# aleCombi/Hedgehog.jl

Hardware: AMD Instinct MI355X
Metric: MC path-steps/sec (Heston Euler-Maruyama, 1e6 paths x 252 steps per GPU) (higher is better)
Workload: dtype f64

## Files before the change

hedgehog.jl_amd/_ffi.py:

```python
from __future__ import annotations

import ctypes as C
import os

HH_MAX_PARTIALS = 8
HH_LSM_PHASE_POW, HH_LSM_PHASE_INIT, HH_LSM_PHASE_STEP = 1, 2, 3
HH_TILE_PATHS = 256
HH_ACC_LEN = 16
HH_MAX_MODELS = 16
HH_ACC_SUM, HH_ACC_SUMSQ, HH_ACC_DSUM, HH_ACC_NPATHS = 0, 1, 2, 10

HH_LOGNORMAL, HH_HESTON = 0, 1
HH_EULER_MARUYAMA, HH_EXACT_LAW, HH_BROADIE_KAYA = 0, 1, 2
HH_NOISE_GENERATE, HH_NOISE_REPLAY = 0, 1
HH_REPLAY_TILE_MAJOR, HH_REPLAY_PATH_MAJOR = 0, 1
HH_PATH_SPOT, HH_PATH_LOG = 0, 1

HH_OK, HH_ERR_INVALID, HH_ERR_UNSUPPORTED, HH_ERR_HIP, HH_ERR_NOMEM, HH_ERR_RCCL, HH_ERR_DEVICE_TIMEOUT = 0, -1, -2, -3, -4, -5, -6
HH_MGPU_AUTO, HH_MGPU_HOST_SUM, HH_MGPU_RCCL = 0, 1, 2
HH_MGPU_REDUCE_HOST, HH_MGPU_REDUCE_RCCL = 0, 1
HH_MGPU_OPT_ENQUEUE = 1
HH_MGPU_ENQUEUE_SERIAL, HH_MGPU_ENQUEUE_THREADS = 0, 1

_dp = C.POINTER(C.c_double)


class hh_model(C.Structure):
    _fields_ = [(n, C.c_double) for n in
                ("S0", "V0", "kappa", "theta", "sigma", "rho", "r_drift", "discount", "T", "strike",
                 "cp")] + \
               [(n, _dp) for n in
                ("dS0", "dV0", "dkappa", "dtheta", "dsigma", "dr_drift", "ddiscount", "dstrike")]


class hh_config(C.Structure):
    _fields_ = [
        ("dynamics", C.c_int32), ("strategy", C.c_int32), ("antithetic", C.c_int32),
        ("em_split", C.c_int32), ("compat_sqrt_alpha", C.c_int32), ("noise_mode", C.c_int32),
        ("replay_layout", C.c_int32), ("seeds_on_device", C.c_int32),
        ("replay_on_device", C.c_int32), ("terminal_on_device", C.c_int32),
        ("n_steps", C.c_uint32), ("n_partials", C.c_uint32),
        ("n_paths", C.c_uint64), ("path_offset", C.c_uint64),
        ("seeds", C.c_void_p), ("replay", C.c_void_p),
        ("bk_n_sigma", C.c_double), ("bk_cf_tol", C.c_double), ("bk_atol", C.c_double),
        ("bk_moment_h", C.c_double),
        ("bk_newton_maxiter", C.c_int32), ("bk_bisect_maxiter", C.c_int32),
        ("bk_root_form", C.c_int32), ("bk_bracket_form", C.c_int32), ("bk_caps", C.c_int32), ("reserved0", C.c_int32),
        ("seeds_len", C.c_uint64), ("replay_len", C.c_uint64),
    ]


class hh_result(C.Structure):
    _fields_ = [
        ("price", C.c_double), ("std_error", C.c_double),
        ("sum_payoff", C.c_double), ("sumsq_payoff", C.c_double),
        ("dprice", C.c_double * HH_MAX_PARTIALS),
        ("n_paths_done", C.c_uint64),
        ("bk_newton_fail", C.c_uint64), ("bk_bisect_fallback", C.c_uint64),
        ("bk_maxguess_fallback", C.c_uint64), ("bk_cf_terms", C.c_uint64),
        ("kernel_ms", C.c_double), ("total_ms", C.c_double),
    ]


class hh_lsm_result(C.Structure):
    _fields_ = [("price", C.c_double), ("std_error", C.c_double), ("n_paths_total", C.c_uint64),
                ("rows_regressed", C.c_uint32), ("rows_skipped", C.c_uint32),
                ("kernel_ms", C.c_double), ("total_ms", C.c_double),
                ("form", C.c_int32), ("persistent_fallbacks", C.c_int32)]


HH_BK_ROOT_SECANT, HH_BK_ROOT_ORDER2 = 0, 1
HH_BK_BRACKET_MIDPOINT, HH_BK_BRACKET_ROOTS = 0, 1
HH_BK_CAPS_AS_WRITTEN, HH_BK_CAPS_ROOTS_DEFAULT = 0, 1
HH_OPT_LSM_FORM = 1
HH_OPT_BK_TERM_CACHE = 2
HH_OPT_GRID_FORM = 3
HH_OPT_LSM_SPIN_TICKS = 4
HH_OPT_FUSE_REDUCE = 5
HH_OPT_GRID_ORDER = 6
HH_OPT_FINISH_SPIN_TICKS = 7
HH_OPT_FINISH_TILE_FIRST = 8
HH_GRID_FORM_PER_DATE, HH_GRID_FORM_BATCHED = 0, 1
HH_CM_GRAD_LEN = 8
HH_LSM_FORM_PER_DATE, HH_LSM_FORM_PERSISTENT, HH_LSM_FORM_AUTO = 0, 1, 2
HH_CRR_MAX_STEPS, HH_CRR_FORM_A_MAX_STEPS = 32768, 2047
HH_CRR_EUROPEAN, HH_CRR_AMERICAN_FORWARD, HH_CRR_AMERICAN_SPOT = 0, 1, 2


class HedgehogMCError(RuntimeError):
    def __init__(self, code: int, msg: str):
        super().__init__(f"hedgehog_mc error {code}: {msg}")
        self.code = code


LIB_PATH = os.environ.get("HEDGEHOG_MC_LIB") or os.path.join(
    os.path.dirname(os.path.abspath(__file__)), "lib", "libhedgehog_mc.so")

_vp = C.c_void_p
SYMBOLS = [
    ("hh_abi_version", C.c_int, []),
    ("hh_ctx_create", C.c_int, [C.POINTER(_vp), C.c_int]),
    ("hh_ctx_destroy", None, [_vp]),
    ("hh_ctx_set_stream", C.c_int, [_vp, _vp]),
    ("hh_ctx_reset_stream", C.c_int, [_vp]),
    ("hh_last_error", C.c_char_p, [_vp]),
    ("hh_ctx_set_option", C.c_int, [_vp, C.c_int32, C.c_int64]),
    ("hh_ctx_check_last", C.c_int, [_vp]),
    ("hh_mc_solve", C.c_int, [_vp, C.POINTER(hh_model), C.POINTER(hh_config), C.POINTER(hh_result), _vp]),
    ("hh_mc_accumulate", C.c_int, [_vp, C.POINTER(hh_model), C.POINTER(hh_config), _vp, _vp]),
    ("hh_mc_solve_multi", C.c_int, [_vp, C.POINTER(hh_model), C.c_uint32, C.POINTER(hh_config), C.POINTER(hh_result), _vp]),
    ("hh_mc_accumulate_multi", C.c_int, [_vp, C.POINTER(hh_model), C.c_uint32, C.POINTER(hh_config), _vp, _vp]),
    ("hh_mc_finalize", C.c_int, [C.POINTER(hh_model), C.POINTER(hh_config), _vp, C.POINTER(hh_result)]),
    ("hh_mc_accumulate_basket", C.c_int, [_vp, C.POINTER(hh_model), C.POINTER(hh_config), _vp, _vp, C.c_uint32, _vp, _vp]),
    ("hh_mc_solve_basket", C.c_int, [_vp, C.POINTER(hh_model), C.POINTER(hh_config), _vp, _vp, C.c_uint32, _vp, _vp]),
    ("hh_carr_madan", C.c_int, [_vp, C.POINTER(hh_model), C.c_int32, C.c_int32, C.c_double, C.c_double, C.POINTER(C.c_double)]),
    ("hh_carr_madan_basket", C.c_int, [_vp, C.POINTER(hh_model), C.c_int32, C.c_int32, C.c_double, C.c_double,
                                       _vp, _vp, _vp, _vp, _vp, C.c_uint32, _vp]),
    ("hh_carr_madan_basket_grad", C.c_int, [_vp, C.POINTER(hh_model), C.c_int32, C.c_int32, C.c_double,
                                            C.c_double, _vp, _vp, _vp, _vp, _vp, C.c_uint32, _vp, _vp]),
    ("hh_crr_solve", C.c_int, [_vp, C.c_int32, C.c_uint32, _vp, _vp, _vp, _vp, _vp, _vp, _vp, C.c_uint32, _vp, _vp]),
    ("hh_lsm_grid_elems", C.c_size_t, [C.c_uint64, C.c_uint32, C.c_int32]),
    ("hh_lsm_solve", C.c_int, [_vp, C.POINTER(hh_model), C.POINTER(hh_config), C.c_int32, C.c_double, C.POINTER(hh_lsm_result), _vp, _vp, _vp]),
    ("hh_lsm_solve_grid", C.c_int, [_vp, C.POINTER(hh_model), _vp, C.c_uint64, C.c_uint32, C.c_int32, C.c_double, C.POINTER(hh_lsm_result), _vp, _vp]),
    ("hh_heston_exact_grid", C.c_int, [_vp, C.POINTER(hh_model), C.POINTER(hh_config), _vp, _vp, C.c_int32, C.POINTER(hh_result)]),
    ("hh_euler_grid", C.c_int, [_vp, C.POINTER(hh_model), C.POINTER(hh_config), C.c_int32, _vp, _vp, C.c_int32, C.POINTER(hh_result)]),
    ("hh_lsm_solve_euler", C.c_int, [_vp, C.POINTER(hh_model), C.POINTER(hh_config), C.c_int32, C.c_int32, C.c_double,
                                     C.POINTER(hh_lsm_result), _vp, _vp, _vp]),
    ("hh_lsm_shard_xchg_elems", C.c_size_t, [C.c_uint32, C.c_int32]),
    ("hh_lsm_shard_begin", C.c_int, [_vp, C.POINTER(hh_model), C.POINTER(hh_config), C.c_int32, C.c_double, _vp]),
    ("hh_lsm_shard_phase", C.c_int, [_vp, C.c_int32, C.c_uint32, _vp, _vp]),
    ("hh_lsm_shard_finish", C.c_int, [_vp, _vp, _vp, _vp, _vp, C.POINTER(C.c_uint32), C.POINTER(C.c_uint32)]),
    ("hh_lsm_finalize", C.c_int, [_vp, C.POINTER(hh_lsm_result)]),
    ("hh_lsm_debug_read", C.c_int, [_vp, C.c_uint64, C.c_uint32, C.c_int32, _vp]),
    ("hh_replay_elems", C.c_size_t, [C.c_uint64, C.c_uint32, C.c_int32]),
    ("hh_replay_pack", C.c_int, [_vp, C.c_int32, C.c_uint64, C.c_uint32, _vp, C.c_int32, _vp]),
    ("hh_wiener_fill", C.c_int, [_vp, C.c_int32, C.c_double, C.c_double, C.c_uint32, C.c_uint64, _vp, C.c_int32, _vp]),
    ("hh_seeds_fingerprint", C.c_uint64, [_vp, C.c_uint64]),
    ("hh_seeds_cache", C.c_int, [_vp, _vp, C.c_uint64, C.c_uint64, C.POINTER(_vp)]),
    ("hh_seeds_cache_stats", C.c_int, [_vp, C.POINTER(C.c_uint64), C.POINTER(C.c_uint64), C.POINTER(C.c_uint64)]),
    ("hh_device_malloc", C.c_int, [_vp, C.c_size_t, C.POINTER(_vp)]),
    ("hh_device_free", C.c_int, [_vp, _vp]),
    ("hh_memcpy_h2d", C.c_int, [_vp, _vp, _vp, C.c_size_t]),
    ("hh_memcpy_d2h", C.c_int, [_vp, _vp, _vp, C.c_size_t]),
    ("hh_ctx_synchronize", C.c_int, [_vp]),
    ("hh_ctx_enable_timing", C.c_int, [_vp, C.c_int32]),
    ("hh_ctx_read_timings", C.c_int, [_vp, _vp, C.c_int32, C.POINTER(C.c_int32)]),
    ("hh_bk_decisions", C.c_int, [_vp, C.c_uint64, _vp, _vp]),
    ("hh_mgpu_create", C.c_int, [C.POINTER(_vp), C.POINTER(C.c_int), C.c_int, C.c_int]),
    ("hh_mgpu_destroy", None, [_vp]),
    ("hh_mgpu_last_error", C.c_char_p, [_vp]),
    ("hh_mgpu_n_devices", C.c_int, [_vp]),
    ("hh_mgpu_reduce_mode", C.c_int, [_vp]),
    ("hh_mgpu_ctx", _vp, [_vp, C.c_int]),
    ("hh_mgpu_selftest", C.c_int, [_vp, C.POINTER(C.c_int32), C.POINTER(C.c_int32)]),
    ("hh_mgpu_rccl_info", C.c_int, [_vp, C.c_char_p, C.c_size_t, C.POINTER(C.c_int32), C.POINTER(C.c_int32)]),
    ("hh_mgpu_set_option", C.c_int, [_vp, C.c_int32, C.c_int64]),
    ("hh_mgpu_enqueue_stats", C.c_int, [_vp, _vp, C.POINTER(C.c_double)]),
    ("hh_mgpu_shard_range", None, [C.c_uint64, C.c_int, C.c_int, C.c_int, C.POINTER(C.c_uint64), C.POINTER(C.c_uint64)]),
    ("hh_mgpu_solve", C.c_int, [_vp, C.POINTER(hh_model), C.POINTER(hh_config), C.POINTER(hh_result), _vp]),
    ("hh_mgpu_solve_shards", C.c_int, [_vp, C.POINTER(hh_model), C.POINTER(hh_config), C.POINTER(hh_result), _vp]),
    ("hh_mgpu_solve_basket", C.c_int, [_vp, C.POINTER(hh_model), C.POINTER(hh_config), _vp, _vp, C.c_uint32, _vp]),
    ("hh_mgpu_solve_multi", C.c_int, [_vp, C.POINTER(hh_model), C.c_uint32, C.POINTER(hh_config), C.POINTER(hh_result)]),
    ("hh_mgpu_lsm_solve", C.c_int, [_vp, C.POINTER(hh_model), C.POINTER(hh_config), C.c_int32, C.c_double,
                                    C.POINTER(hh_lsm_result), _vp, _vp]),
# ... 324 lines not shown
```

hedgehog.jl_amd/csrc/hh_api.hip:

```cpp
#include <cmath>
#include <cstdarg>
#include <cstdio>
#include <cstring>
#include <mutex>
#include <vector>

#include "hh_kernels.h"

#include "hh_ctx.h"

namespace {

const char* const kNoCtx = "hedgehog_mc: no context";

int ncomp_of(int dynamics) { return dynamics == HH_HESTON ? 2 : 1; }

constexpr uint64_t kMaxPaths = (1ull << 32) - 256;
constexpr uint32_t kMaxEulerSteps = 4u * 65535u;
constexpr uint32_t kMaxGridSteps = 65534u;

static bool bk_law_ok(const hh_model* m, double dt) {
  const double s2 = m->sigma * m->sigma;
  const double d = 4.0 * m->kappa * m->theta / s2;
  if (!(d >= 1e-8 && d <= 1e6)) return false;
  const double em1 = -std::expm1(-m->kappa * dt);
  const double lam_per_v = 4.0 * m->kappa * std::exp(-m->kappa * dt) / (s2 * em1);
  const double cscale = s2 * em1 / (4.0 * m->kappa);
  const double nuk = 4.0 * m->kappa * std::exp(-0.5 * m->kappa * dt) / s2 / em1;
  return std::isfinite(lam_per_v) && lam_per_v >= 0.0 && std::isfinite(cscale) && cscale > 0.0 &&
         std::isfinite(nuk) && nuk > 0.0 && std::isfinite(m->kappa * (1.0 + std::exp(-m->kappa * dt)) / em1);
}

int validate(hh_ctx* ctx, const hh_model* m, const hh_config* c) {
  if (!m || !c) return fail(ctx, HH_ERR_INVALID, "model/config is NULL");
  if (c->n_paths == 0) return fail(ctx, HH_ERR_INVALID, "n_paths must be >= 1");
  if (c->n_paths > kMaxPaths)
    return fail(ctx, HH_ERR_INVALID, "n_paths too large (max 2^32 - 256 per call; shard the ensemble)");
  if (c->strategy == HH_EULER_MARUYAMA && c->n_steps > kMaxEulerSteps)
    return fail(ctx, HH_ERR_INVALID, "n_steps too large (max %u)", kMaxEulerSteps);
  if (c->n_partials > HH_MAX_PARTIALS)
    return fail(ctx, HH_ERR_INVALID, "n_partials %u > HH_MAX_PARTIALS", c->n_partials);
  const bool logn = c->dynamics == HH_LOGNORMAL, hest = c->dynamics == HH_HESTON;
  if (!logn && !hest) return fail(ctx, HH_ERR_INVALID, "unknown dynamics %d", c->dynamics);
  const bool ok = (logn && (c->strategy == HH_EULER_MARUYAMA || c->strategy == HH_EXACT_LAW)) ||
                  (hest && (c->strategy == HH_EULER_MARUYAMA || c->strategy == HH_BROADIE_KAYA));
  if (!ok)
    return fail(ctx, HH_ERR_UNSUPPORTED, "no simulation method for dynamics %d with strategy %d",
                c->dynamics, c->strategy);
  if (!(m->S0 > 0.0) || !std::isfinite(m->S0)) return fail(ctx, HH_ERR_INVALID, "S0 must be > 0");
  if (!(m->T > 0.0) || !std::isfinite(m->T)) return fail(ctx, HH_ERR_INVALID, "T must be > 0");
  if (m->cp != 1.0 && m->cp != -1.0) return fail(ctx, HH_ERR_INVALID, "cp must be +1 or -1");
  if (hest && !(std::fabs(m->rho) <= 1.0)) return fail(ctx, HH_ERR_INVALID, "|rho| must be <= 1");
  if (!std::isfinite(m->sigma) || !std::isfinite(m->r_drift) || !std::isfinite(m->discount) ||
      !std::isfinite(m->strike) ||
      (hest && (!std::isfinite(m->V0) || !std::isfinite(m->kappa) || !std::isfinite(m->theta))))
    return fail(ctx, HH_ERR_INVALID, "model scalars must be finite");
  if (c->strategy == HH_EULER_MARUYAMA && c->n_steps == 0)
    return fail(ctx, HH_ERR_INVALID, "n_steps must be >= 1 for EulerMaruyama");
  if (c->strategy == HH_BROADIE_KAYA) {
    if (c->antithetic)
      return fail(ctx, HH_ERR_UNSUPPORTED, "HestonBroadieKaya has no antithetic form");
    if (c->n_partials)
      return fail(ctx, HH_ERR_UNSUPPORTED, "HestonBroadieKaya does not carry dual partials");
    if (m->sigma == 0.0 || m->kappa == 0.0 || !(m->V0 > 0.0))
      return fail(ctx, HH_ERR_INVALID, "HestonBroadieKaya needs sigma != 0, kappa != 0, V0 > 0");
    if ((c->bk_root_form != HH_BK_ROOT_SECANT && c->bk_root_form != HH_BK_ROOT_ORDER2) ||
        (c->bk_bracket_form != HH_BK_BRACKET_MIDPOINT && c->bk_bracket_form != HH_BK_BRACKET_ROOTS) ||
        (c->bk_caps != HH_BK_CAPS_AS_WRITTEN && c->bk_caps != HH_BK_CAPS_ROOTS_DEFAULT))
      return fail(ctx, HH_ERR_INVALID, "bk_root_form, bk_bracket_form, bk_caps: 0 or 1 each (hedgehog_mc.h)");
    if (!bk_law_ok(m, m->T))
      return fail(ctx, HH_ERR_INVALID, "HestonBroadieKaya needs 1e-8 <= d = 4 kappa theta / sigma^2 <= 1e6 "
                                       "(Bessel order d/2 - 1 strictly above -1, tables up to order 5e5) and "
                                       "finite transition constants (|kappa T| < 700)");
  }
  const bool euler = c->strategy == HH_EULER_MARUYAMA;
  if (c->noise_mode == HH_NOISE_REPLAY) {
    if (!c->replay) return fail(ctx, HH_ERR_INVALID, "REPLAY needs a replay buffer");
    if (((uintptr_t)c->replay & 15u) != 0)
      return fail(ctx, HH_ERR_INVALID, "replay buffer must be 16-byte aligned");
    if (c->replay_len) {
      uint64_t need = c->n_paths;
      if (c->strategy == HH_BROADIE_KAYA) need = 3 * c->n_paths;
      if (euler)
        need = c->replay_layout == HH_REPLAY_PATH_MAJOR
                   ? c->n_paths * (uint64_t)c->n_steps * (uint64_t)ncomp_of(c->dynamics)
                   : (uint64_t)hh::tiles_for(c->n_paths) * c->n_steps * ncomp_of(c->dynamics) *
                         hh::kTile;
      if (c->replay_len < need)
        return fail(ctx, HH_ERR_INVALID, "replay buffer holds %llu elements, %llu needed",
                    (unsigned long long)c->replay_len, (unsigned long long)need);
    }
  } else if (c->noise_mode == HH_NOISE_GENERATE) {
    if (!c->seeds) return fail(ctx, HH_ERR_INVALID, "GENERATE needs seeds");
    const uint64_t need = euler ? c->n_paths : 1;
    if (c->seeds_len && c->seeds_len < need)
      return fail(ctx, HH_ERR_INVALID, "Number of seeds (%llu) must be >= number of trajectories (%llu)",
                  (unsigned long long)c->seeds_len, (unsigned long long)need);
  } else {
    return fail(ctx, HH_ERR_INVALID, "unknown noise_mode %d", c->noise_mode);
  }
  return HH_OK;
}

int ensure_poisoned(hh_ctx* ctx, size_t need) {
  if (need <= ctx->frecords_cap) return HH_OK;
  int rc = ensure(ctx, ctx->frecords, ctx->frecords_cap, need);
  if (rc) return rc;
  static_assert((hh::kPoison >> 32) == (hh::kPoison & 0xffffffffull), "hipMemsetD32 writes the pattern");
  HH_HIP(ctx, hipMemsetD32Async((hipDeviceptr_t)ctx->frecords, (int)(hh::kPoison & 0xffffffffull),
                                ctx->frecords_cap * 2, ctx->stream));
  return HH_OK;
}

constexpr uint32_t kFuseAutoMaxRecords = 512, kFuseAutoMinSteps = 32;
bool fuse_for(const hh_ctx* ctx, const hh_config* c) {
  if (ctx->fuse_reduce != 2) return ctx->fuse_reduce == 1;
  return hh::sim_records(*c) <= kFuseAutoMaxRecords || (c->strategy == HH_EULER_MARUYAMA && c->n_steps >= kFuseAutoMinSteps);
}

void fused_controls(const hh_ctx* ctx, hh::DevicePtrs& p) {
  p.finish_state = ctx->finish_state;
  p.finish_spin_ticks = ctx->finish_spin_ticks;
  p.finish_tile_first = ctx->finish_tile_first;
}

int recover_finish(hh_ctx* ctx) {
  unsigned int state = 0;
  HH_HIP(ctx, hipStreamSynchronize(ctx->stream));
  HH_HIP(ctx, hipMemcpy(&state, ctx->finish_state, sizeof(state), hipMemcpyDeviceToHost));
  if (state == 0u) return HH_OK;
  if (ctx->frecords_cap)
    HH_HIP(ctx, hipMemsetD32Async((hipDeviceptr_t)ctx->frecords, (int)(hh::kPoison & 0xffffffffull),
                                  ctx->frecords_cap * 2, ctx->stream));
  HH_HIP(ctx, hipMemsetAsync(ctx->finish_state, 0, 2 * sizeof(unsigned int), ctx->stream));
  HH_HIP(ctx, hipStreamSynchronize(ctx->stream));
  const long long ticks = ctx->finish_spin_ticks < 0 ? (long long)hh::kFinishSpinTicksDefault : ctx->finish_spin_ticks;
  return fail(ctx, HH_ERR_DEVICE_TIMEOUT,
              "the record reduction inside a simulation kernel gave up: a workgroup's record had not arrived after %lld "
              "ticks of the 100 MHz clock (a queue preempted for that long, or a workgroup that died); the sums of that "
              "solve, and of solves queued behind it, are lost — the context's record buffer has been reset and the "
              "context can be used again", ticks);
}

int finalize_failed(hh_ctx* ctx, int rc) {
  const int rf = recover_finish(ctx);
  return rf ? rf : fail(ctx, rc, "finalize failed: the accumulator holds no trajectories");
}

size_t replay_elems(uint64_t n_paths, uint32_t n_steps, int dynamics) {
  return (size_t)hh::tiles_for(n_paths) * n_steps * ncomp_of(dynamics) * hh::kTile;
}

int solve_times(hh_ctx* ctx, const WallClock& clock, double* kernel_ms, double* total_ms) {
  float ms = 0.f;
  HH_HIP(ctx, hipEventElapsedTime(&ms, ctx->ev0, ctx->ev1));
  *kernel_ms = ms;
  *total_ms = clock.ms();
  return HH_OK;
}

void payoff_moments(const double* acc, double n, double* mean, double* var) {
  *mean = acc[HH_ACC_SUM] / n;
  *var = n > 1.0 ? (acc[HH_ACC_SUMSQ] - n * *mean * *mean) / (n - 1.0) : 0.0;
  if (!(*var > 0.0)) *var = 0.0;
}

}

extern "C" {

int hh_abi_version(void) { return HH_ABI_VERSION; }

int hh_ctx_create(hh_ctx** out, int device_id) {
  if (!out) return HH_ERR_INVALID;
  *out = nullptr;
  int n = 0;
  if (hipGetDeviceCount(&n) != hipSuccess || n <= 0) return HH_ERR_HIP;
  if (device_id < 0 || device_id >= n) return HH_ERR_INVALID;
  hh_ctx* ctx = new (std::nothrow) hh_ctx();
  if (!ctx) return HH_ERR_NOMEM;
  ctx->device = device_id;
  if (hipSetDevice(device_id) != hipSuccess ||
      hipStreamCreateWithFlags(&ctx->own_stream, hipStreamNonBlocking) != hipSuccess ||
      hipEventCreate(&ctx->ev0) != hipSuccess || hipEventCreate(&ctx->ev1) != hipSuccess ||
      hipEventCreateWithFlags(&ctx->ev_switch, hipEventDisableTiming) != hipSuccess ||
      hipEventCreateWithFlags(&ctx->ev_stage, hipEventDisableTiming) != hipSuccess ||
      hipMalloc((void**)&ctx->accum, HH_ACC_LEN * sizeof(double)) != hipSuccess ||
      hipMalloc((void**)&ctx->finish_state, 2 * sizeof(unsigned int)) != hipSuccess ||
      hipMemset(ctx->finish_state, 0, 2 * sizeof(unsigned int)) != hipSuccess ||
      hipHostMalloc((void**)&ctx->accum_host, (HH_ACC_LEN + 8) * sizeof(double), hipHostMallocDefault) !=
          hipSuccess) {
    hh_ctx_destroy(ctx);
    return HH_ERR_HIP;
  }
  ctx->stream = ctx->own_stream;
  *out = ctx;
  return HH_OK;
}

void hh_ctx_destroy(hh_ctx* ctx) {
  if (!ctx) return;
  (void)hipSetDevice(ctx->device);
  if (ctx->own_stream) (void)hipStreamSynchronize(ctx->own_stream);
  (void)hipDeviceSynchronize();
  if (ctx->records) (void)hipFree(ctx->records);
  if (ctx->seeds) (void)hipFree(ctx->seeds);
  if (ctx->replay) (void)hipFree(ctx->replay);
  if (ctx->replay_src) (void)hipFree(ctx->replay_src);
  if (ctx->terminal) (void)hipFree(ctx->terminal);
  if (ctx->terminal_d) (void)hipFree(ctx->terminal_d);
  if (ctx->payoffs) (void)hipFree(ctx->payoffs);
  if (ctx->basket_records) (void)hipFree(ctx->basket_records);
  if (ctx->basket_accum) (void)hipFree(ctx->basket_accum);
  if (ctx->bk_scratch) (void)hipFree(ctx->bk_scratch);
  if (ctx->bk_sort) (void)hipFree(ctx->bk_sort);
  if (ctx->lsm_grid) (void)hipFree(ctx->lsm_grid);
  if (ctx->heston_var) (void)hipFree(ctx->heston_var);
  if (ctx->lsm_val) (void)hipFree(ctx->lsm_val);
  if (ctx->lsm_tau) (void)hipFree(ctx->lsm_tau);
  if (ctx->lsm_scratch) (void)hipFree(ctx->lsm_scratch);
  for (auto& e : ctx->seed_cache)
    if (e.dev) (void)hipFree(e.dev);
  if (ctx->accum) (void)hipFree(ctx->accum);
  if (ctx->frecords) (void)hipFree(ctx->frecords);
  if (ctx->finish_state) (void)hipFree(ctx->finish_state);
  if (ctx->accum_host) (void)hipHostFree(ctx->accum_host);
  for (auto& pr : ctx->tev)
    for (auto& e : pr)
      if (e) (void)hipEventDestroy(e);
  if (ctx->ev_switch) (void)hipEventDestroy(ctx->ev_switch);
  if (ctx->ev_stage) (void)hipEventDestroy(ctx->ev_stage);
  if (ctx->ev0) (void)hipEventDestroy(ctx->ev0);
  if (ctx->ev1) (void)hipEventDestroy(ctx->ev1);
  if (ctx->own_stream) (void)hipStreamDestroy(ctx->own_stream);
  delete ctx;
}

static int switch_stream(hh_ctx* ctx, hipStream_t next) {
  if (next == ctx->stream) return HH_OK;
  HH_HIP(ctx, hipSetDevice(ctx->device));
  HH_HIP(ctx, hipEventRecord(ctx->ev_switch, ctx->stream));
  HH_HIP(ctx, hipStreamWaitEvent(next, ctx->ev_switch, 0));
  ctx->stream = next;
  return HH_OK;
}

int hh_ctx_set_stream(hh_ctx* ctx, void* hip_stream) {
  if (!ctx) return HH_ERR_INVALID;
  std::lock_guard<std::recursive_mutex> lock__(ctx->mu);
  return switch_stream(ctx, (hipStream_t)hip_stream);
}

int hh_ctx_reset_stream(hh_ctx* ctx) {
  if (!ctx) return HH_ERR_INVALID;
  std::lock_guard<std::recursive_mutex> lock__(ctx->mu);
  return switch_stream(ctx, ctx->own_stream);
}

const char* hh_last_error(const hh_ctx* ctx) { return ctx ? ctx->err : kNoCtx; }

int hh_ctx_set_option(hh_ctx* ctx, int32_t option, int64_t value) {
  if (!ctx) return HH_ERR_INVALID;
  std::lock_guard<std::recursive_mutex> lock__(ctx->mu);
  switch (option) {
    case HH_OPT_LSM_FORM:
      if (value != HH_LSM_FORM_PER_DATE && value != HH_LSM_FORM_PERSISTENT && value != HH_LSM_FORM_AUTO)
        return fail(ctx, HH_ERR_INVALID, "HH_OPT_LSM_FORM: 0 (launch per date), 1 (one launch) or 2 (auto)");
      ctx->lsm_form = (int)value;
      return HH_OK;
    case HH_OPT_BK_TERM_CACHE:
      if (value < 8 || value > 1024)
        return fail(ctx, HH_ERR_INVALID, "HH_OPT_BK_TERM_CACHE: 8 .. 1024 series terms per trajectory");
      ctx->bk_term_cache = (int)value;
      return HH_OK;
    case HH_OPT_LSM_SPIN_TICKS:
      if (value < -1) return fail(ctx, HH_ERR_INVALID, "HH_OPT_LSM_SPIN_TICKS: ticks of the 100 MHz clock, 0 = give up at once, -1 = default");
      ctx->lsm_spin_ticks = value;
      return HH_OK;
    case HH_OPT_GRID_FORM:
      if (value != HH_GRID_FORM_PER_DATE && value != HH_GRID_FORM_BATCHED)
        return fail(ctx, HH_ERR_INVALID, "HH_OPT_GRID_FORM: 0 (one chain per date) or 1 (dates batched)");
      ctx->grid_form = (int)value;
      return HH_OK;
    case HH_OPT_GRID_ORDER:
      if (value != 0 && value != 1)
        return fail(ctx, HH_ERR_INVALID, "HH_OPT_GRID_ORDER: 0 (a chain's pairs in their natural order) or 1 (sorted by their Bessel arguments)");
      ctx->grid_order = (int)value;
      return HH_OK;
    case HH_OPT_FINISH_SPIN_TICKS:
      if (value < -1) return fail(ctx, HH_ERR_INVALID, "HH_OPT_FINISH_SPIN_TICKS: ticks of the 100 MHz clock, 0 = give up at once, -1 = default");
      ctx->finish_spin_ticks = value;
      return HH_OK;
    case HH_OPT_FINISH_TILE_FIRST:
      if (value != 0 && value != 1) return fail(ctx, HH_ERR_INVALID, "HH_OPT_FINISH_TILE_FIRST: 0 (the last tile's workgroup adds the records) or 1 (the first one's)");
      ctx->finish_tile_first = (int)value;
      return HH_OK;
    case HH_OPT_FUSE_REDUCE:
      if (value < 0 || value > 2)
        return fail(ctx, HH_ERR_INVALID, "HH_OPT_FUSE_REDUCE: 0 (a second kernel reduces the records), 1 (the simulation kernel does) or 2 (by size)");
      ctx->fuse_reduce = (int)value;
      return HH_OK;
    default:
      return fail(ctx, HH_ERR_INVALID, "unknown option %d", option);
  }
}

int hh_ctx_synchronize(hh_ctx* ctx) {
  if (!ctx) return HH_ERR_INVALID;
  std::lock_guard<std::recursive_mutex> lock__(ctx->mu);
  HH_HIP(ctx, hipSetDevice(ctx->device));
  HH_HIP(ctx, hipStreamSynchronize(ctx->stream));
  return HH_OK;
}

size_t hh_replay_elems(uint64_t n_paths, uint32_t n_steps, int32_t dynamics) {
  return replay_elems(n_paths, n_steps, dynamics);
}

int hh_replay_pack(hh_ctx* ctx, int32_t dynamics, uint64_t n_paths, uint32_t n_steps,
                   const double* src, int32_t src_on_device, double* dst) {
  if (!ctx) return HH_ERR_INVALID;
  std::lock_guard<std::recursive_mutex> lock__(ctx->mu);
  if (!src || !dst || n_paths == 0 || n_steps == 0 || n_paths > kMaxPaths || n_steps > kMaxEulerSteps)
    return fail(ctx, HH_ERR_INVALID, "hh_replay_pack: bad arguments");
  HH_HIP(ctx, hipSetDevice(ctx->device));
  const int nc = ncomp_of(dynamics);
  const double* src_dev = src;
  if (!src_on_device) {
    const size_t n = (size_t)n_paths * n_steps * nc;
    const int rc = stage_host(ctx, ctx->replay_src, ctx->replay_src_cap, n, src, n, &src_dev);
    if (rc) return rc;
  }
  HH_HIP(ctx, hh::launch_replay_pack(nc, n_paths, n_steps, src_dev, dst, ctx->stream));
  return release_host_operands(ctx);
}

int hh_wiener_fill(hh_ctx* ctx, int32_t dynamics, double rho, double T, uint32_t n_steps,
                   uint64_t n_paths, const uint64_t* seeds, int32_t seeds_on_device, double* dst) {
  if (!ctx) return HH_ERR_INVALID;
  std::lock_guard<std::recursive_mutex> lock__(ctx->mu);
  if (!seeds || !dst || n_paths == 0 || n_steps == 0 || !(T > 0.0) || !(std::fabs(rho) <= 1.0) ||
      n_paths > kMaxPaths || n_steps > kMaxEulerSteps)
    return fail(ctx, HH_ERR_INVALID, "hh_wiener_fill: bad arguments");
  HH_HIP(ctx, hipSetDevice(ctx->device));
  const uint64_t* seeds_dev = seeds;
  if (!seeds_on_device) {
    const int rc = stage_host(ctx, ctx->seeds, ctx->seeds_cap, (size_t)n_paths, seeds, (size_t)n_paths, &seeds_dev);
    if (rc) return rc;
  }
  const double dt = T / (double)n_steps;
  HH_HIP(ctx, hh::launch_wiener_fill(dynamics, rho, std::sqrt(dt), n_steps, n_paths, seeds_dev, dst,
                                     ctx->stream));
  return release_host_operands(ctx);
}

static int stage_noise(hh_ctx* ctx, const hh_config* c, hh::DevicePtrs& p, bool tile_major_only) {
  int rc = HH_OK;
  const bool bk = c->strategy == HH_BROADIE_KAYA;
  if (c->noise_mode == HH_NOISE_GENERATE) {
    const size_t need = (c->strategy == HH_EULER_MARUYAMA) ? (size_t)c->n_paths : 1;
    if (c->seeds_on_device)
      p.seeds = c->seeds;
    else if ((rc = stage_host(ctx, ctx->seeds, ctx->seeds_cap, need, c->seeds, need, &p.seeds)))
      return rc;
  } else if (bk) {
    const size_t n3 = (size_t)3 * c->n_paths;
    if (c->replay_on_device)
      p.replay = c->replay;
    else if ((rc = stage_host(ctx, ctx->replay, ctx->replay_cap, n3, c->replay, n3, &p.replay)))
      return rc;
  } else {
    const uint32_t steps = (c->strategy == HH_EULER_MARUYAMA) ? c->n_steps : 1;
    const int dyn = (c->strategy == HH_EULER_MARUYAMA) ? c->dynamics : HH_LOGNORMAL;
    const size_t tile_elems = replay_elems(c->n_paths, steps, dyn);
    if (c->replay_layout == HH_REPLAY_PATH_MAJOR && c->strategy == HH_EULER_MARUYAMA && !tile_major_only &&
        hh::replay_direct_path_major(steps, ncomp_of(dyn))) {
      const size_t n = (size_t)c->n_paths * steps * ncomp_of(dyn);
      if (c->replay_on_device)
        p.replay = c->replay;
      else if ((rc = stage_host(ctx, ctx->replay_src, ctx->replay_src_cap, n, c->replay, n, &p.replay)))
        return rc;
      p.replay_path_major = true;
    } else if (c->replay_layout == HH_REPLAY_PATH_MAJOR) {
      rc = ensure(ctx, ctx->replay, ctx->replay_cap, tile_elems);
      if (rc) return rc;
      rc = hh_replay_pack(ctx, dyn, c->n_paths, steps, c->replay, c->replay_on_device, ctx->replay);
      if (rc) return rc;
      p.replay = ctx->replay;
    } else if (c->replay_layout == HH_REPLAY_TILE_MAJOR) {
      if (c->replay_on_device) {
        p.replay = c->replay;
      } else {
        const size_t host_elems =
            (c->strategy == HH_EULER_MARUYAMA) ? tile_elems : (size_t)c->n_paths;
        rc = stage_host(ctx, ctx->replay, ctx->replay_cap, tile_elems, c->replay, host_elems, &p.replay);
        if (rc) return rc;
      }
    } else {
      return fail(ctx, HH_ERR_INVALID, "unknown replay_layout %d", c->replay_layout);
    }
  }

  return HH_OK;
}

static int run_simulation(hh_ctx* ctx, const hh_model* m, const hh_config* c, double* terminal,
                          bool need_terminal_dev, double** terminal_dev_out, double* accum_dev = nullptr,
                          bool* reduced = nullptr) {
  int rc = HH_OK;
  const uint32_t n_tiles = hh::tiles_for(c->n_paths);
  const bool bk = c->strategy == HH_BROADIE_KAYA;
  rc = ensure(ctx, ctx->records, ctx->records_cap,
              (size_t)(bk ? hh::bk_record_count(c->n_paths) : n_tiles) * hh::kRecStride);
  if (rc) return rc;

  hh::DevicePtrs p{};
  p.records = ctx->records;
  const bool fuse = accum_dev && !bk && fuse_for(ctx, c);
  if (fuse) {
    if ((rc = ensure_poisoned(ctx, (size_t)n_tiles * hh::kRecStride))) return rc;
    p.records = ctx->frecords;
    p.accum = accum_dev;
    fused_controls(ctx, p);
  }
  if (reduced) *reduced = fuse || bk;
  if (bk) {
    rc = ensure_bk_scratch(ctx, hh::bk_scratch_bytes(c->n_paths, ctx->bk_term_cache));
    if (rc) return rc;
    p.accum = accum_dev ? accum_dev : ctx->accum;
    p.bk_scratch = ctx->bk_scratch;
    p.bk_table_key = &ctx->bk_table_key;
    p.bk_term_cache = ctx->bk_term_cache;
    ctx->bk_last_n = c->n_paths;
    ctx->bk_last_cache = ctx->bk_term_cache;
  }

  if ((rc = stage_noise(ctx, c, p, false))) return rc;

  const size_t n_term = (size_t)c->n_paths * (c->antithetic ? 2 : 1);
  if (terminal && c->terminal_on_device) {
    p.terminal = terminal;
  } else if (terminal || need_terminal_dev) {
    rc = ensure(ctx, ctx->terminal, ctx->terminal_cap, n_term);
    if (rc) return rc;
    p.terminal = ctx->terminal;
  }
  const int n_active = c->n_partials ? hh::count_active_partials(*m, *c) : 0;
  if (need_terminal_dev && n_active) {
    rc = ensure(ctx, ctx->terminal_d, ctx->terminal_d_cap,
                n_term * (size_t)hh::pad_partials((uint32_t)n_active));
    if (rc) return rc;
    p.terminal_d = ctx->terminal_d;
  }
  if (terminal_dev_out) *terminal_dev_out = p.terminal;

  if (ctx->timing) HH_HIP(ctx, hipEventRecord(ctx->tev[ctx->t_count % hh_ctx::kTimingSlots][0], ctx->stream));
  if (c->strategy == HH_BROADIE_KAYA)
    HH_HIP(ctx, hh::launch_bk(*m, *c, p, ctx->stream));
  else
    HH_HIP(ctx, hh::launch_simulation(*m, *c, p, ctx->stream));
  return HH_OK;
}

static int end_timing(hh_ctx* ctx) {
  if (ctx->timing) {
    HH_HIP(ctx, hipEventRecord(ctx->tev[ctx->t_count % hh_ctx::kTimingSlots][1], ctx->stream));
    ++ctx->t_count;
  }
  return HH_OK;
}

static int copy_back_terminal(hh_ctx* ctx, const hh_config* c, double* terminal) {
  if (terminal && !c->terminal_on_device) {
    const size_t n_term = (size_t)c->n_paths * (c->antithetic ? 2 : 1);
    HH_HIP(ctx, hipMemcpyAsync(terminal, ctx->terminal, n_term * sizeof(double),
                               hipMemcpyDeviceToHost, ctx->stream));
    HH_HIP(ctx, hipStreamSynchronize(ctx->stream));
  }
  return HH_OK;
}

int hh_mc_accumulate(hh_ctx* ctx, const hh_model* m, const hh_config* c, double* accum_dev,
                     double* terminal) {
  if (!ctx) return HH_ERR_INVALID;
  std::lock_guard<std::recursive_mutex> lock__(ctx->mu);
  int rc = validate(ctx, m, c);
  if (rc) return rc;
  if (!accum_dev) return fail(ctx, HH_ERR_INVALID, "accum_dev is NULL");
  HH_HIP(ctx, hipSetDevice(ctx->device));
  bool reduced = false;
  rc = run_simulation(ctx, m, c, terminal, false, nullptr, accum_dev, &reduced);
  if (rc) return rc;
  if (!reduced)
    HH_HIP(ctx, hh::launch_reduce_records(ctx->records, hh::sim_records(*c), (double)c->n_paths, accum_dev, ctx->stream, 1, m, c));
  if ((rc = end_timing(ctx))) return rc;
  if ((rc = release_host_operands(ctx))) return rc;
  return copy_back_terminal(ctx, c, terminal);
}

static int next_pass(int remaining) {
  if (remaining <= hh::kMaxModelsPerPass) return remaining;
  return remaining == hh::kMaxModelsPerPass + 1 ? hh::kMaxModelsPerPass - 1 : hh::kMaxModelsPerPass;
}

int hh_mc_accumulate_multi(hh_ctx* ctx, const hh_model* models, uint32_t n_models, const hh_config* c,
                           double* accum_dev, double* const* terminals) {
  if (!ctx) return HH_ERR_INVALID;
  std::lock_guard<std::recursive_mutex> lock__(ctx->mu);
  if (!models || n_models == 0 || n_models > HH_MAX_MODELS)
    return fail(ctx, HH_ERR_INVALID, "hh_mc_accumulate_multi: 1 .. %d models", HH_MAX_MODELS);
  if (!accum_dev) return fail(ctx, HH_ERR_INVALID, "accum_dev is NULL");
  int rc;
  for (uint32_t k = 0; k < n_models; ++k)
    if ((rc = validate(ctx, &models[k], c))) return rc;
  if (c->n_partials)
    return fail(ctx, HH_ERR_UNSUPPORTED, "several models in one pass carry no dual partials (n_partials must be 0)");
  if (n_models == 1) return hh_mc_accumulate(ctx, models, c, accum_dev, terminals ? terminals[0] : nullptr);
  HH_HIP(ctx, hipSetDevice(ctx->device));
  if (c->strategy == HH_BROADIE_KAYA) {
    const uint32_t count = hh::bk_record_count(c->n_paths);
    if ((rc = ensure(ctx, ctx->records, ctx->records_cap, 2 * (size_t)count * hh::kRecStride))) return rc;
    std::vector<int> leader(n_models, -1);
    for (uint32_t k = 0; k < n_models; ++k)
      for (uint32_t j = 0; j < k; ++j)
        if (leader[j] < 0 && hh::bk_same_chain(models[j], models[k])) {
          leader[k] = (int)j;
          break;
        }
    for (uint32_t k = 0; k < n_models; ++k) {
      if (leader[k] >= 0) continue;
      if ((rc = hh_mc_accumulate(ctx, &models[k], c, accum_dev + (size_t)k * HH_ACC_LEN, terminals ? terminals[k] : nullptr)))
        return rc;
      for (uint32_t f = k + 1; f < n_models; ++f) {
        if (leader[f] != (int)k) continue;
        double* terminal = terminals ? terminals[f] : nullptr;
        hh::DevicePtrs p{};
        p.records = ctx->records + (size_t)count * hh::kRecStride;
        p.bk_scratch = ctx->bk_scratch;
        p.bk_term_cache = ctx->bk_term_cache;
        if (terminal && c->terminal_on_device) {
          p.terminal = terminal;
        } else if (terminal) {
          if ((rc = ensure(ctx, ctx->terminal, ctx->terminal_cap, (size_t)c->n_paths))) return rc;
          p.terminal = ctx->terminal;
        }
        if (ctx->timing) HH_HIP(ctx, hipEventRecord(ctx->tev[ctx->t_count % hh_ctx::kTimingSlots][0], ctx->stream));
        HH_HIP(ctx, hh::launch_bk_refinish(models[f], *c, p, ctx->records, ctx->stream));
        HH_HIP(ctx, hh::launch_reduce_records(p.records, count, (double)c->n_paths, accum_dev + (size_t)f * HH_ACC_LEN,
                                              ctx->stream, 1, &models[f], c, false,
                                              hh::bk_live_records(ctx->bk_scratch, c->n_paths)));
        if ((rc = end_timing(ctx))) return rc;
        if ((rc = copy_back_terminal(ctx, c, terminal))) return rc;
      }
    }
    return HH_OK;
  }
  const uint32_t n_tiles = hh::tiles_for(c->n_paths);
  const size_t rec_elems = (size_t)n_tiles * hh::kRecStride;
  const bool fuse = fuse_for(ctx, c);
  if (fuse) rc = ensure_poisoned(ctx, (size_t)n_models * rec_elems);
  else rc = ensure(ctx, ctx->records, ctx->records_cap, (size_t)n_models * rec_elems);
  if (rc) return rc;
  hh::DevicePtrs base{};
  if (fuse) fused_controls(ctx, base);
  if ((rc = stage_noise(ctx, c, base, true))) return rc;
  const size_t n_term = (size_t)c->n_paths * (c->antithetic ? 2 : 1);
  bool any_host_terminal = false;
  if (terminals && !c->terminal_on_device) {
    for (uint32_t k = 0; k < n_models; ++k) any_host_terminal = any_host_terminal || terminals[k] != nullptr;
    if (any_host_terminal && (rc = ensure(ctx, ctx->terminal, ctx->terminal_cap, (size_t)n_models * n_term))) return rc;
  }
  std::vector<hh::DevicePtrs> p(n_models, base);
  for (uint32_t k = 0; k < n_models; ++k) {
    p[k].records = (fuse ? ctx->frecords : ctx->records) + (size_t)k * rec_elems;
    p[k].accum = fuse ? accum_dev + (size_t)k * HH_ACC_LEN : nullptr;
    double* t = terminals ? terminals[k] : nullptr;
    p[k].terminal = !t ? nullptr : c->terminal_on_device ? t : ctx->terminal + (size_t)k * n_term;
  }
  if (ctx->timing) HH_HIP(ctx, hipEventRecord(ctx->tev[ctx->t_count % hh_ctx::kTimingSlots][0], ctx->stream));
  for (uint32_t k0 = 0; k0 < n_models;) {
    const int take = next_pass((int)(n_models - k0));
    HH_HIP(ctx, hh::launch_simulation_multi(models + k0, take, *c, p.data() + k0, ctx->stream));
    if (!fuse)
      for (int k = 0; k < take; ++k)
        HH_HIP(ctx, hh::launch_reduce_records(p[k0 + k].records, hh::sim_records(*c), (double)c->n_paths,
                                              accum_dev + (size_t)(k0 + k) * HH_ACC_LEN, ctx->stream, 1, &models[k0 + k], c));
    k0 += (uint32_t)take;
  }
  if ((rc = end_timing(ctx))) return rc;
  if ((rc = release_host_operands(ctx))) return rc;
  if (any_host_terminal) {
    for (uint32_t k = 0; k < n_models; ++k)
      if (terminals[k])
        HH_HIP(ctx, hipMemcpyAsync(terminals[k], p[k].terminal, n_term * sizeof(double), hipMemcpyDeviceToHost, ctx->stream));
    HH_HIP(ctx, hipStreamSynchronize(ctx->stream));
  }
  return HH_OK;
}

int hh_mc_solve_multi(hh_ctx* ctx, const hh_model* models, uint32_t n_models, const hh_config* c, hh_result* out,
                      double* const* terminals) {
  if (!ctx) return HH_ERR_INVALID;
  std::lock_guard<std::recursive_mutex> lock__(ctx->mu);
  if (!out || !models || n_models == 0 || n_models > HH_MAX_MODELS)
    return fail(ctx, HH_ERR_INVALID, "hh_mc_solve_multi: 1 .. %d models and their results", HH_MAX_MODELS);
  const WallClock clock;
  HH_HIP(ctx, hipSetDevice(ctx->device));
  const size_t n_acc = (size_t)n_models * HH_ACC_LEN;
  int rc = ensure(ctx, ctx->basket_accum, ctx->basket_accum_cap, n_acc);
  if (rc) return rc;
  HH_HIP(ctx, hipEventRecord(ctx->ev0, ctx->stream));
  if ((rc = hh_mc_accumulate_multi(ctx, models, n_models, c, ctx->basket_accum, terminals))) return rc;
  HH_HIP(ctx, hipEventRecord(ctx->ev1, ctx->stream));
  double host[HH_MAX_MODELS * HH_ACC_LEN];
  HH_HIP(ctx, hipMemcpyAsync(host, ctx->basket_accum, n_acc * sizeof(double), hipMemcpyDeviceToHost, ctx->stream));
  HH_HIP(ctx, hipStreamSynchronize(ctx->stream));
  double kernel_ms, total_ms;
  if ((rc = solve_times(ctx, clock, &kernel_ms, &total_ms))) return rc;
  rc = finalize_results(models, 1, c, host, n_models, kernel_ms, total_ms, out);
  return rc ? finalize_failed(ctx, rc) : HH_OK;
}

int hh_mc_accumulate_basket(hh_ctx* ctx, const hh_model* m, const hh_config* c,
                            const double* strikes, const double* cps, uint32_t n_payoffs,
                            double* accum_dev, double* terminal) {
  if (!ctx) return HH_ERR_INVALID;
  std::lock_guard<std::recursive_mutex> lock__(ctx->mu);
  int rc = validate(ctx, m, c);
  if (rc) return rc;
  if (!accum_dev || !strikes || !cps || n_payoffs == 0 || n_payoffs > 65535)
    return fail(ctx, HH_ERR_INVALID, "hh_mc_accumulate_basket: bad arguments");
  for (uint32_t k = 0; k < n_payoffs; ++k)
    if (cps[k] != 1.0 && cps[k] != -1.0) return fail(ctx, HH_ERR_INVALID, "cp must be +1 or -1");
  if (m->dstrike)
    return fail(ctx, HH_ERR_UNSUPPORTED, "strike partials are not carried through a basket");
  HH_HIP(ctx, hipSetDevice(ctx->device));
  double* term_dev = nullptr;
  rc = run_simulation(ctx, m, c, terminal, true, &term_dev);
  if (rc) return rc;

  hh::BasketArgs b{};
  b.n_paths = c->n_paths;
  b.n_chunks = hh::basket_chunks(c->n_paths);
  b.antithetic = c->antithetic;
  std::vector<double> payoffs(strikes, strikes + n_payoffs);
  payoffs.insert(payoffs.end(), cps, cps + n_payoffs);
  const double* payoffs_dev = nullptr;
  rc = stage_host(ctx, ctx->payoffs, ctx->payoffs_cap, payoffs.size(), payoffs.data(), payoffs.size(), &payoffs_dev);
  if (rc) return rc;
  rc = ensure(ctx, ctx->basket_records, ctx->basket_records_cap,
              (size_t)n_payoffs * b.n_chunks * hh::kRecStride);
  if (rc) return rc;
  b.terminal = term_dev;
  const int n_active = c->n_partials ? hh::count_active_partials(*m, *c) : 0;
  b.terminal_d = n_active ? ctx->terminal_d : nullptr;
  b.strikes = payoffs_dev;
  b.cps = payoffs_dev + n_payoffs;
  b.records = ctx->basket_records;
  HH_HIP(ctx, hh::launch_basket_payoffs(b, n_payoffs, (uint32_t)n_active, ctx->stream));
  HH_HIP(ctx, hh::launch_reduce_records(ctx->basket_records, b.n_chunks, (double)c->n_paths,
                                        accum_dev, ctx->stream, n_payoffs, m, c, true));
  if (c->strategy == HH_BROADIE_KAYA)
    HH_HIP(ctx, hh::launch_copy_bk_counters(ctx->accum, accum_dev, n_payoffs, ctx->stream));
  if ((rc = end_timing(ctx))) return rc;
  if ((rc = release_host_operands(ctx))) return rc;
  return copy_back_terminal(ctx, c, terminal);
}

int hh_mc_solve_basket(hh_ctx* ctx, const hh_model* m, const hh_config* c, const double* strikes,
                       const double* cps, uint32_t n_payoffs, hh_result* out, double* terminal) {
  if (!ctx) return HH_ERR_INVALID;
  std::lock_guard<std::recursive_mutex> lock__(ctx->mu);
  if (!out) return fail(ctx, HH_ERR_INVALID, "result is NULL");
  const WallClock clock;
  HH_HIP(ctx, hipSetDevice(ctx->device));
  const size_t n_acc = (size_t)n_payoffs * HH_ACC_LEN;
  int rc = ensure(ctx, ctx->basket_accum, ctx->basket_accum_cap, n_acc);
  if (rc) return rc;
  HH_HIP(ctx, hipEventRecord(ctx->ev0, ctx->stream));
  rc = hh_mc_accumulate_basket(ctx, m, c, strikes, cps, n_payoffs, ctx->basket_accum, terminal);
  if (rc) return rc;
  HH_HIP(ctx, hipEventRecord(ctx->ev1, ctx->stream));
  std::vector<double> host(n_acc);
  HH_HIP(ctx, hipMemcpyAsync(host.data(), ctx->basket_accum, n_acc * sizeof(double),
                             hipMemcpyDeviceToHost, ctx->stream));
  HH_HIP(ctx, hipStreamSynchronize(ctx->stream));
  double kernel_ms, total_ms;
  if ((rc = solve_times(ctx, clock, &kernel_ms, &total_ms))) return rc;
  rc = finalize_results(m, 0, c, host.data(), n_payoffs, kernel_ms, total_ms, out);
  return rc ? finalize_failed(ctx, rc) : HH_OK;
}

int hh_mc_finalize(const hh_model* m, const hh_config* c, const double* acc, hh_result* out) {
  if (!m || !c || !acc || !out) return HH_ERR_INVALID;
  const double n = acc[HH_ACC_NPATHS];
  if (!(n >= 1.0)) return HH_ERR_INVALID;
  double mean, var;
  payoff_moments(acc, n, &mean, &var);
  out->sum_payoff = acc[HH_ACC_SUM];
  out->sumsq_payoff = acc[HH_ACC_SUMSQ];
  out->price = m->discount * mean;
  out->std_error = m->discount * std::sqrt(var / n);
  for (uint32_t k = 0; k < HH_MAX_PARTIALS; ++k) {
    double d = 0.0;
    if (k < c->n_partials) {
      const double dD = m->ddiscount ? m->ddiscount[k] : 0.0;
      d = dD * mean + m->discount * (acc[HH_ACC_DSUM + k] / n);
    }
    out->dprice[k] = d;
  }
  out->n_paths_done = (uint64_t)n;
  out->bk_newton_fail = (uint64_t)acc[HH_ACC_BK_NEWTON_FAIL];
  out->bk_bisect_fallback = (uint64_t)acc[HH_ACC_BK_BISECT];
  out->bk_maxguess_fallback = (uint64_t)acc[HH_ACC_BK_MAXGUESS];
  out->bk_cf_terms = (uint64_t)acc[HH_ACC_BK_CF_TERMS];
  return HH_OK;
}

int hh_mc_solve(hh_ctx* ctx, const hh_model* m, const hh_config* c, hh_result* out,
                double* terminal) {
  if (!ctx) return HH_ERR_INVALID;
  std::lock_guard<std::recursive_mutex> lock__(ctx->mu);
  if (!out) return fail(ctx, HH_ERR_INVALID, "result is NULL");
  const WallClock clock;
  std::memset(out, 0, sizeof(*out));
  HH_HIP(ctx, hipSetDevice(ctx->device));
  HH_HIP(ctx, hipEventRecord(ctx->ev0, ctx->stream));
  int rc = hh_mc_accumulate(ctx, m, c, ctx->accum, terminal);
  if (rc) return rc;
  HH_HIP(ctx, hipEventRecord(ctx->ev1, ctx->stream));
  HH_HIP(ctx, hipMemcpyAsync(ctx->accum_host, ctx->accum, HH_ACC_LEN * sizeof(double),
                             hipMemcpyDeviceToHost, ctx->stream));
  HH_HIP(ctx, hipStreamSynchronize(ctx->stream));
  rc = hh_mc_finalize(m, c, ctx->accum_host, out);
  if (rc) return finalize_failed(ctx, rc);
  return solve_times(ctx, clock, &out->kernel_ms, &out->total_ms);
}

int hh_ctx_check_last(hh_ctx* ctx) {
  if (!ctx) return HH_ERR_INVALID;
  std::lock_guard<std::recursive_mutex> lock__(ctx->mu);
  HH_HIP(ctx, hipSetDevice(ctx->device));
  return recover_finish(ctx);
}

int hh_bk_decisions(hh_ctx* ctx, uint64_t n_paths, uint32_t* decisions, uint32_t* series_len) {
  if (!ctx) return HH_ERR_INVALID;
  std::lock_guard<std::recursive_mutex> lock__(ctx->mu);
  if (!ctx->bk_scratch || ctx->bk_last_n == 0 || n_paths != ctx->bk_last_n)
    return fail(ctx, HH_ERR_INVALID, "hh_bk_decisions: the last Broadie-Kaya solve of this context had %llu trajectories",
                (unsigned long long)ctx->bk_last_n);
  HH_HIP(ctx, hipSetDevice(ctx->device));
  const uint32_t *dec = nullptr, *len = nullptr;
  hh::bk_diag_ptrs(ctx->bk_scratch, n_paths, ctx->bk_last_cache, &dec, &len);
  if (decisions)
    HH_HIP(ctx, hipMemcpyAsync(decisions, dec, n_paths * sizeof(uint32_t), hipMemcpyDeviceToHost, ctx->stream));
  if (series_len)
    HH_HIP(ctx, hipMemcpyAsync(series_len, len, n_paths * sizeof(uint32_t), hipMemcpyDeviceToHost, ctx->stream));
  HH_HIP(ctx, hipStreamSynchronize(ctx->stream));
  return HH_OK;
}

int hh_carr_madan(hh_ctx* ctx, const hh_model* m, int32_t dynamics, int32_t compat_sqrt_alpha,
                  double alpha, double bound, double* price_out) {
  if (!ctx) return HH_ERR_INVALID;
  std::lock_guard<std::recursive_mutex> lock__(ctx->mu);
  if (!m || !price_out) return fail(ctx, HH_ERR_INVALID, "hh_carr_madan: NULL argument");
  if (dynamics != HH_LOGNORMAL && dynamics != HH_HESTON)
    return fail(ctx, HH_ERR_INVALID, "unknown dynamics %d", dynamics);
  if (!(m->S0 > 0.0) || !(m->strike > 0.0) || !(m->T > 0.0) || !(alpha > 0.0) || !(bound > 0.0) ||
      (m->cp != 1.0 && m->cp != -1.0) || (dynamics == HH_HESTON && m->sigma == 0.0))
    return fail(ctx, HH_ERR_INVALID, "hh_carr_madan: bad scalars");
  HH_HIP(ctx, hipSetDevice(ctx->device));
  HH_HIP(ctx, hh::launch_carr_madan(*m, dynamics, compat_sqrt_alpha, alpha, bound, ctx->accum,
                                    ctx->stream));
  HH_HIP(ctx, hipMemcpyAsync(ctx->accum_host, ctx->accum, sizeof(double), hipMemcpyDeviceToHost,
                             ctx->stream));
  HH_HIP(ctx, hipStreamSynchronize(ctx->stream));
  const double call = ctx->accum_host[0];
  *price_out = m->cp > 0.0 ? call : call - m->S0 + m->strike * m->discount;
  return HH_OK;
}

static int cm_upload_payoffs(hh_ctx* ctx, const char* who, const double* strikes, const double* cps, const double* Ts,
                             const double* r_drifts, const double* discounts, size_t n, size_t out_len,
                             std::vector<double>& host) {
  for (size_t k = 0; k < n; ++k) {
    if (!(strikes[k] > 0.0) || !(Ts[k] > 0.0) || (cps[k] != 1.0 && cps[k] != -1.0) ||
        !std::isfinite(r_drifts[k]) || !(discounts[k] > 0.0))
      return fail(ctx, HH_ERR_INVALID, "%s: payoff %zu: strike, T, discount > 0, cp = +-1", who, k);
    host[k] = std::log(strikes[k]);
    host[n + k] = Ts[k];
    host[2 * n + k] = r_drifts[k];
    host[3 * n + k] = discounts[k];
  }
  HH_HIP(ctx, hipSetDevice(ctx->device));
  int rc = ensure(ctx, ctx->payoffs, ctx->payoffs_cap, 4 * n + out_len);
  if (rc) return rc;
  HH_HIP(ctx, hipMemcpyAsync(ctx->payoffs, host.data(), 4 * n * sizeof(double), hipMemcpyHostToDevice,
                             ctx->stream));
  return HH_OK;
}

int hh_carr_madan_basket(hh_ctx* ctx, const hh_model* m, int32_t dynamics, int32_t compat_sqrt_alpha,
                         double alpha, double bound, const double* strikes, const double* cps,
                         const double* Ts, const double* r_drifts, const double* discounts,
                         uint32_t n_payoffs, double* prices_out) {
  if (!ctx) return HH_ERR_INVALID;
  std::lock_guard<std::recursive_mutex> lock__(ctx->mu);
  if (!m || !strikes || !cps || !Ts || !r_drifts || !discounts || !prices_out)
    return fail(ctx, HH_ERR_INVALID, "hh_carr_madan_basket: NULL argument");
  if (dynamics != HH_LOGNORMAL && dynamics != HH_HESTON)
    return fail(ctx, HH_ERR_INVALID, "unknown dynamics %d", dynamics);
  if (n_payoffs == 0 || n_payoffs > (1u << 20))
    return fail(ctx, HH_ERR_INVALID, "hh_carr_madan_basket: 1 .. 2^20 payoffs per call");
  if (!(m->S0 > 0.0) || !(alpha > 0.0) || !(bound > 0.0) || (dynamics == HH_HESTON && m->sigma == 0.0))
    return fail(ctx, HH_ERR_INVALID, "hh_carr_madan_basket: bad scalars");
// ... 636 lines not shown
```

hedgehog.jl_amd/csrc/hh_bk.hip:

```cpp
#include <algorithm>
#include <atomic>
#include <cmath>

#include "hh_bessel.h"
#include "hh_kernels.h"
#include "hh_math.h"
#include "hh_reduce.h"
#include "hh_rng.h"

namespace hh {

namespace {

constexpr double kPi = kBesselPi;
constexpr double kTwoPi = kBesselTwoPi, kInvTwoPi = 0.15915494309189533577;
constexpr double kInvPi = 0.31830988618379067154, kTwoOverPi = 0.63661977236758134308;

#ifndef HH_BK_COMPLEX_SETUP
#define HH_BK_COMPLEX_SETUP 0
#endif
#ifndef HH_BK_SERIAL_LADDER
#define HH_BK_SERIAL_LADDER 0
#endif

// ... 974 lines not shown
    if (stage == kLadderLo) {
      fa = f;
      x = xb;
      stage = kLadderHi;
      continue;
    }
    if (stage == kLadderHi) {
      fb = f;
      if (fa * fb > 0.0) {
        acc[4] += 1.0;
        dec |= kDecMaxGuess;
        break;
      }
      acc[3] += 1.0;
      dec |= kDecBisect;
      x = roots_bisect ? roots_middle(xa, xb) : 0.5 * (xa + xb);
      if (cap_bisect <= 0 || (roots_bisect && !(xa < x && x < xb))) break;
      stage = kBisect;
      continue;
    }
    ++iters;
    bool stop;
    if (roots_bisect) {
      if (f == 0.0) {
        out_set = true;
      } else if (sign_of(fa) * sign_of(f) < 0) {
        xb = x;
        fb = f;
      } else {
        xa = x;
        fa = f;
      }
      const double mid = roots_middle(xa, xb);
      stop = out_set || (int)iters >= cap_bisect || !(xa < mid && mid < xb);
      if (!out_set) x = stop ? mid : mid;
    } else {
      if (f == 0.0) {
        xa = xb = x;
      } else if ((f < 0.0) == (fa < 0.0)) {
        xa = x;
        fa = f;
      } else {
        xb = x;
      }
      x = 0.5 * (xa + xb);
      stop = f == 0.0 || xb - xa <= p.atol || (int)iters >= cap_bisect;
    }
    if (stop) {
      dec |= (iters & 0xffu) << kDecItersShift;
      break;
    }
  }
  if (roots_bisect && (dec & kDecBisect) && !out_set) x = fabs(fa) < fabs(fb) ? xa : xb;
  const double IV = x;
  p.diag[path] = dec;
  p.diag[p.draw_stride + path] = (uint32_t)s.cache.j_stop;
  acc[5] += n_terms;
  const double pay = bk_finish_path(p, path, IV);
  acc[0] += pay;
  acc[1] = fma(pay, pay, acc[1]);
}

template <class Fn>
__device__ __forceinline__ void for_long_tiles(const unsigned long long* __restrict__ long_mask, uint32_t n_tiles,
                                               uint32_t b, Fn&& fn) {
  __shared__ unsigned char hit[kTile];
  for (uint32_t t0 = b; t0 < n_tiles; t0 += (uint32_t)kHeavyGrid * kTile) {
    const uint32_t t = t0 + threadIdx.x * (uint32_t)kHeavyGrid;
    unsigned long long any = 0ull;
    if (t < n_tiles) {
#pragma unroll
      for (int w = 0; w < kTile / 64; ++w) any |= long_mask[(size_t)t * (kTile / 64) + w];
    }
    __syncthreads();
    hit[threadIdx.x] = any != 0ull;
    __syncthreads();
    for (uint32_t i = 0; i < (uint32_t)kTile; ++i)
      if (hit[i]) fn(t0 + i * (uint32_t)kHeavyGrid);
  }
}

__global__ __launch_bounds__(kTile) void bk_tail_kernel(const BkArgs* __restrict__ args, const BkTables* __restrict__ tabs,
                                                        uint32_t n_tiles, double n_paths, double* __restrict__ accum,
                                                        uint32_t* __restrict__ cnt, const double* __restrict__ records) {
  const uint32_t b = blockIdx.x, tid = threadIdx.x;
  __shared__ double sm[257];
  const uint32_t n_long_v = __hip_atomic_load(cnt, __ATOMIC_RELAXED, __HIP_MEMORY_SCOPE_AGENT);
  double out = 0.0;
  if (b < (uint32_t)kRecStride) out = sum_slot(records, n_tiles, (int)b, sm);
  const uint32_t n_long = (uint32_t)__builtin_amdgcn_readfirstlane((int)n_long_v);
  uint32_t n_rec = n_tiles;
  if (n_long != 0u) {
    const BkArgs& p = *args;
    double acc[6] = {0, 0, 0, 0, 0, 0};
    for_long_tiles(p.long_mask, n_tiles, b, [&](uint32_t tile) {
      const uint64_t path = (uint64_t)tile * kTile + tid;
      if ((p.long_mask[(size_t)tile * (kTile / 64) + (tid >> 6)] >> (tid & 63u)) & 1ull)
        tail_whole_trajectory(p, tabs->t, tabs->coef, path, acc);
    });
    bk_store_record(acc, p.records + (size_t)(n_tiles + b) * kRecStride);
    __syncthreads();
    if (tid == 0) {
      __builtin_amdgcn_fence(__ATOMIC_RELEASE, "agent");
      asm volatile("s_waitcnt vmcnt(0)" ::: "memory");
      __hip_atomic_fetch_add(cnt + 2, 1u, __ATOMIC_RELAXED, __HIP_MEMORY_SCOPE_AGENT);
    }
    if (b >= (uint32_t)kRecStride) return;
    if (tid == 0) {
      while (__hip_atomic_load(cnt + 2, __ATOMIC_RELAXED, __HIP_MEMORY_SCOPE_AGENT) != (uint32_t)kHeavyGrid)
        __builtin_amdgcn_s_sleep(8);
      __builtin_amdgcn_fence(__ATOMIC_ACQUIRE, "agent");
      asm volatile("s_waitcnt vmcnt(0)" ::: "memory");
      if (__hip_atomic_fetch_add(cnt + 3, 1u, __ATOMIC_RELAXED, __HIP_MEMORY_SCOPE_AGENT) == (uint32_t)kRecStride - 1u) {
        __hip_atomic_store(cnt, 0u, __ATOMIC_RELAXED, __HIP_MEMORY_SCOPE_AGENT);
        __hip_atomic_store(cnt + 2, 0u, __ATOMIC_RELAXED, __HIP_MEMORY_SCOPE_AGENT);
        __hip_atomic_store(cnt + 3, 0u, __ATOMIC_RELAXED, __HIP_MEMORY_SCOPE_AGENT);
      }
    }
    __syncthreads();
    n_rec = n_tiles + (uint32_t)kHeavyGrid;
    out = sum_slot(records, n_rec, (int)b, sm);
  } else if (b >= (uint32_t)kRecStride) {
    return;
  }
  if (tid == 0) {
    accum[b] = b == (uint32_t)HH_ACC_NPATHS ? n_paths : out;
    if (b == 0u) cnt[1] = n_rec;
  }
}

__global__ __launch_bounds__(kTile) void bk_refinish_kernel(const BkArgs p, const double* __restrict__ rec0, uint32_t n_tiles) {
  const uint32_t b = blockIdx.x, tid = threadIdx.x;
  if (b >= p.counters[1]) return;
  double acc[6] = {0, 0, 0, 0, 0, 0};
  if (b < n_tiles) {
    const uint64_t path = (uint64_t)b * kTile + tid;
    const bool left = (p.long_mask[(size_t)b * (kTile / 64) + (tid >> 6)] >> (tid & 63u)) & 1ull;
    if (path < p.n_paths && !left) {
      const double pay = bk_finish_path(p, path, p.iv_keep[path]);
      acc[0] = pay;
      acc[1] = pay * pay;
    }
  } else {
    for_long_tiles(p.long_mask, n_tiles, b - n_tiles, [&](uint32_t tile) {
      const uint64_t path = (uint64_t)tile * kTile + tid;
      if ((p.long_mask[(size_t)tile * (kTile / 64) + (tid >> 6)] >> (tid & 63u)) & 1ull) {
        const double pay = bk_finish_path(p, path, p.iv_keep[path]);
        acc[0] += pay;
        acc[1] = fma(pay, pay, acc[1]);
      }
    });
  }
  double* rec = p.records + (size_t)b * kRecStride;
  bk_store_record(acc, rec);
  if (tid == 0) {
    const double* r0 = rec0 + (size_t)b * kRecStride;
    rec[HH_ACC_BK_NEWTON_FAIL] = r0[HH_ACC_BK_NEWTON_FAIL];
    rec[HH_ACC_BK_BISECT] = r0[HH_ACC_BK_BISECT];
    rec[HH_ACC_BK_MAXGUESS] = r0[HH_ACC_BK_MAXGUESS];
    rec[HH_ACC_BK_CF_TERMS] = r0[HH_ACC_BK_CF_TERMS];
  }
}

__global__ __launch_bounds__(64) void bk_tables_kernel(const BkBessel t, BkTables* __restrict__ dst, double kappa,
                                                        double sigma2, double T, double eta_k, double zeta_k) {
  for (int j = (int)threadIdx.x; j <= kCoefTerms; j += 64) dst->coef[j] = kTwoOverPi / (double)j;
  if (threadIdx.x != 0) return;
  dst->zero = chf_zero(kappa, sigma2, T, eta_k, zeta_k);
  const double* src = reinterpret_cast<const double*>(&t);
  double* out = reinterpret_cast<double*>(dst->t);
  static_assert(sizeof(BkBessel) == sizeof(dst->t), "the Bessel tables of BkTables");
#pragma unroll
  for (size_t i = 0; i < sizeof(BkBessel) / sizeof(double); ++i) out[i] = src[i];
}

__global__ __launch_bounds__(256) void fill_rows_kernel(double* __restrict__ spot0,
                                                        double* __restrict__ var0, uint64_t n,
                                                        double S0, double V0) {
  const uint64_t i = (uint64_t)blockIdx.x * 256 + threadIdx.x;
  if (i < n) {
    spot0[i] = S0;
    var0[i] = V0;
  }
}

constexpr int kSortRun = 1024;
constexpr int kSortWaves = kTile / 64;
static_assert(kSortRun % 64 == 0, "whole rounds of a wave");

__global__ __launch_bounds__(kTile) void grid_sort_count_kernel(const uint8_t* __restrict__ keys, uint32_t n, uint32_t n_runs,
                                                                uint32_t* __restrict__ counts) {
  __shared__ uint32_t hist[kSortWaves][256];
  const uint32_t wave = threadIdx.x >> 6, lane = threadIdx.x & 63u, run = blockIdx.x * kSortWaves + wave;
  for (uint32_t d = lane; d < 256u; d += 64u) hist[wave][d] = 0u;
  __syncthreads();
  if (run < n_runs) {
    const uint32_t base = run * (uint32_t)kSortRun;
    constexpr int kRounds = kSortRun / 64;
    uint32_t key[kRounds];
#pragma unroll
    for (int r = 0; r < kRounds; ++r) {
      const uint32_t i = base + (uint32_t)r * 64u + lane;
      key[r] = i < n ? (uint32_t)keys[i] : 256u;
    }
#pragma unroll
    for (int r = 0; r < kRounds; ++r)
      if (key[r] < 256u) atomicAdd(&hist[wave][key[r]], 1u);
  }
  __syncthreads();
// ... 142 lines not shown
  a.rho = m.rho; a.V0 = m.V0; a.T = m.T; a.logS0 = log(m.S0); a.r = m.r_drift;
  a.strike = m.strike; a.cp = m.cp;
  const double em1 = -expm1(-m.kappa * m.T);
  a.d = 4.0 * m.kappa * m.theta / a.sigma2;
  a.lam_num = 4.0 * m.kappa * exp(-m.kappa * m.T);
  a.lam_den = a.sigma2 * em1;
  a.cscale = a.sigma2 * em1 / (4.0 * m.kappa);
  a.nu = 0.5 * a.d - 1.0;
  a.zeta_k = em1 / m.kappa;
  a.eta_k = m.kappa * (1.0 + exp(-m.kappa * m.T)) / em1;
  a.nuk_factor = 4.0 * m.kappa * exp(-0.5 * m.kappa * m.T) / a.sigma2 / em1;
  if (!(a.d > 0.0) || !std::isfinite(a.d) || !(a.lam_num * m.V0 / a.lam_den >= 0.0))
    return (int)hipErrorInvalidValue;
  a.n_int = a.nu >= 1.0 ? (int)floor(a.nu) : 0;
  a.n_sigma = c.bk_n_sigma > 0.0 ? c.bk_n_sigma : 5.0;
  a.cf_tol = c.bk_cf_tol > 0.0 ? c.bk_cf_tol : 1e-3;
  a.atol = c.bk_atol > 0.0 ? c.bk_atol : 1e-4;
  a.moment_h = c.bk_moment_h > 0.0 ? c.bk_moment_h : 1e-2;
  a.newton_maxiter = c.bk_newton_maxiter > 0 ? c.bk_newton_maxiter : 10;
  a.bisect_maxiter = c.bk_bisect_maxiter > 0 ? c.bk_bisect_maxiter : 100;
  a.root_form = c.bk_root_form;
  a.bracket_form = c.bk_bracket_form;
  a.caps = c.bk_caps;
  a.n_paths = n_chain;
  a.path_offset = c.path_offset;
  a.seeds = ptr.seeds;
  a.terminal = ptr.terminal;
  a.records = ptr.records;
  const uint32_t n_tiles = tiles_for(n_chain);
  const size_t lanes = (size_t)n_tiles * kTile;
  unsigned char* base = reinterpret_cast<unsigned char*>(ptr.bk_scratch);
  a.long_mask = reinterpret_cast<unsigned long long*>(base);
  L.n_tiles = n_tiles;
  a.slot_busy = reinterpret_cast<uint32_t*>(base + bk_lines_offset(n_tiles));
  a.counters = a.slot_busy + 8 * 32;
  a.args_dev = base + bk_args_offset(n_tiles);
  L.tabs_dev = reinterpret_cast<BkTables*>(base + bk_tables_offset(n_tiles));
  a.tabs_dev = L.tabs_dev;
  a.n_tiles = n_tiles;
  a.cache_cap = phi_cache_cap(ptr.bk_term_cache);
  a.phi_cache = reinterpret_cast<double*>(base + bk_flags_bytes(n_tiles));
  a.cache_stride = bk_cache_columns(n_tiles);
  a.static_slots = n_tiles <= (uint32_t)kSlots ? 1u : 0u;
  a.draws = a.phi_cache + a.cache_stride * (size_t)a.cache_cap;
  a.iv_store = a.draws + 4 * lanes;
  a.diag = reinterpret_cast<uint32_t*>(a.iv_store + lanes);
  a.draw_stride = lanes;
  return 0;
}

int bk_tables(const BkArgs& a, const BkLayout& L, const DevicePtrs& ptr, hipStream_t s, bool upload_tables) {
  if (ptr.bk_table_key)
    upload_tables = !(ptr.bk_table_key->where == L.tabs_dev && ptr.bk_table_key->nu == a.nu &&
                      ptr.bk_table_key->kappa == a.kappa && ptr.bk_table_key->sigma2 == a.sigma2 &&
                      ptr.bk_table_key->T == a.T);
  if (upload_tables) {
    (void)hipMemsetAsync(a.slot_busy, 0, kSlotBitmapBytes, s);
    BkBessel tabs;
    if (!bessel_table(a.nu, tabs.t[0]) || !bessel_table(a.nu - a.n_int, tabs.t[1]))
      return (int)hipErrorInvalidValue;
    hipLaunchKernelGGL(bk_tables_kernel, dim3(1), dim3(64), 0, s, tabs, L.tabs_dev, a.kappa, a.sigma2, a.T, a.eta_k,
                       a.zeta_k);
    if (ptr.bk_table_key) *ptr.bk_table_key = BkTableKey{L.tabs_dev, a.nu, a.kappa, a.sigma2, a.T};
  }
  return 0;
}

uint32_t cf_resident_workgroups() {
  static std::atomic<uint32_t> cache[64];
  int dev = 0;
  if (hipGetDevice(&dev) != hipSuccess || dev < 0 || dev >= 64) return 0u;
  uint32_t v = cache[dev].load(std::memory_order_relaxed);
  if (v == 0u) {
    int cus = 0, per_cu = 0;
    if (hipDeviceGetAttribute(&cus, hipDeviceAttributeMultiprocessorCount, dev) != hipSuccess ||
        hipOccupancyMaxActiveBlocksPerMultiprocessor(&per_cu, bk_cf_kernel<0, 1>, kTile, 0) != hipSuccess || cus <= 0 || per_cu <= 0)
      return 0u;
    v = (uint32_t)cus * (uint32_t)per_cu;
    cache[dev].store(v, std::memory_order_relaxed);
  }
  return v;
}

void bk_chain(const BkArgs& a0, const BkLayout& L, hipStream_t s, double* accum, double n_acc, int draw = 0) {
  BkArgs a = a0;
  const uint32_t resident = cf_resident_workgroups();
  a.drain_tile = resident != 0u && L.n_tiles > resident ? L.n_tiles - resident : 0xffffffffu;
  const dim3 b(kTile), g(L.n_tiles);
  const BkTables* tabs = static_cast<const BkTables*>(L.tabs_dev);
  if (a.order)
    hipLaunchKernelGGL(bk_cf_kernel<1>, g, b, 0, s, a, tabs);
  else if (draw == 1)
    hipLaunchKernelGGL((bk_cf_kernel<0, 1>), g, b, 0, s, a, tabs);
  else if (draw == 2)
    hipLaunchKernelGGL((bk_cf_kernel<0, 2>), g, b, 0, s, a, tabs);
  else
    hipLaunchKernelGGL(bk_cf_kernel<0>, g, b, 0, s, a, tabs);
  hipLaunchKernelGGL(bk_tail_kernel, dim3(kHeavyGrid), b, 0, s, static_cast<const BkArgs*>(a.args_dev), tabs, L.n_tiles,
                     n_acc, accum, a.counters, static_cast<const double*>(a.records));
}

}

int launch_bk(const hh_model& m, const hh_config& c, const DevicePtrs& ptr, hipStream_t s,
              const BkTransition* tr, bool upload_tables) {
  if (!ptr.accum) return (int)hipErrorInvalidValue;
  BkArgs a{};
  BkLayout L{};
  if (tr) {
    a.in_spot = tr->in_spot; a.in_var = tr->in_var;
    a.out_spot = tr->out_spot; a.out_var = tr->out_var;
    a.step = tr->step;
  }
  int rc = bk_prepare(m, c, ptr, c.n_paths, a, L);
  if (rc) return rc;
  a.replay = c.noise_mode == HH_NOISE_REPLAY ? ptr.replay : nullptr;
  if (!tr) a.iv_keep = a.iv_store;
  if ((rc = bk_tables(a, L, ptr, s, upload_tables))) return rc;
  int draw = a.replay ? 2 : 1;
  if (a.in_var) {
    if (a.replay) return (int)hipErrorInvalidValue;
    hipLaunchKernelGGL(bk_draw_kernel, dim3(L.n_tiles), dim3(kTile), 0, s, a);
    draw = 0;
  }
  bk_chain(a, L, s, ptr.accum, (double)c.n_paths, draw);
  return (int)hipGetLastError();
}

bool bk_same_chain(const hh_model& a, const hh_model& b) {
  return a.kappa == b.kappa && a.theta == b.theta && a.sigma == b.sigma && a.V0 == b.V0 && a.T == b.T;
}

int launch_bk_refinish(const hh_model& m, const hh_config& c, const DevicePtrs& ptr, const double* rec0, hipStream_t s) {
  BkArgs a{};
  BkLayout L{};
  const int rc = bk_prepare(m, c, ptr, c.n_paths, a, L);
  if (rc) return rc;
  a.iv_keep = a.iv_store;
  hipLaunchKernelGGL(bk_refinish_kernel, dim3(L.n_tiles + (uint32_t)kHeavyGrid), dim3(kTile), 0, s, a, rec0, L.n_tiles);
  return (int)hipGetLastError();
}

uint32_t bk_grid_dates_per_chain(uint64_t n_paths, uint32_t n_steps, int term_cache) {
  (void)term_cache;
  const uint64_t pairs_max = (uint64_t)1 << 22;
  const uint64_t per = n_paths ? pairs_max / n_paths : 1;
  if (per <= 1) return 1;
  const uint64_t chains = (n_steps + per - 1) / per;
  return (uint32_t)((n_steps + chains - 1) / chains);
}

void bk_diag_ptrs(const void* scratch, uint64_t n_paths, int term_cache, const uint32_t** decisions,
                  const uint32_t** series_len) {
  const size_t n_tiles = tiles_for(n_paths), lanes = n_tiles * kTile;
  const unsigned char* base = reinterpret_cast<const unsigned char*>(scratch);
  const double* cache = reinterpret_cast<const double*>(base + bk_flags_bytes(n_tiles));
  const double* draws = cache + bk_cache_columns(n_tiles) * (size_t)phi_cache_cap(term_cache);
  const uint32_t* diag = reinterpret_cast<const uint32_t*>(draws + 5 * lanes);
  *decisions = diag;
  *series_len = diag + lanes;
}

static uint32_t grid_sort_runs(uint64_t n_chain) { return (uint32_t)((n_chain + kSortRun - 1) / kSortRun); }
size_t bk_grid_sort_bytes(uint64_t n_chain) {
  const size_t lanes = (size_t)tiles_for(n_chain) * kTile;
  return lanes * sizeof(uint32_t) + ((size_t)256 * grid_sort_runs(n_chain) + 256) * sizeof(uint32_t) + lanes + 256;
}

int launch_bk_grid(const hh_model& m, const hh_config& c, const DevicePtrs& ptr, hipStream_t s,
                   double* spot_rows, double* var_rows, uint32_t k0, uint32_t n_dates, bool upload_tables) {
  if (!ptr.accum) return (int)hipErrorInvalidValue;
  BkArgs a{};
  BkLayout L{};
  const uint64_t n_row = c.n_paths, n_chain = n_row * n_dates;
  int rc = bk_prepare(m, c, ptr, n_chain, a, L);
  if (rc) return rc;
  a.in_var = var_rows;
  a.step = k0;
  a.iv_out = a.iv_store;
  if ((rc = bk_tables(a, L, ptr, s, upload_tables))) return rc;
  const dim3 rows(tiles_for(n_row)), b(kTile);
  const bool ordered = ptr.bk_sort && n_chain >= kGridOrderMinPairs && n_chain < (1ull << 31);
  const size_t lanes = (size_t)L.n_tiles * kTile;
  const uint32_t n_runs = grid_sort_runs(n_chain);
  uint32_t* perm = reinterpret_cast<uint32_t*>(ptr.bk_sort);
  uint32_t* counts = perm + lanes;
  uint32_t* totals = counts + (size_t)256 * n_runs;
  uint8_t* keys = reinterpret_cast<uint8_t*>(totals + 256);
  hipLaunchKernelGGL(bk_draw_grid_kernel, rows, b, 0, s, a, n_row, k0, n_dates, var_rows, ordered ? keys : nullptr);
  if (ordered) {
    const dim3 sort_grid((n_runs + kSortWaves - 1) / kSortWaves);
    hipLaunchKernelGGL(grid_sort_count_kernel, sort_grid, b, 0, s, static_cast<const uint8_t*>(keys), (uint32_t)n_chain,
                       n_runs, counts);
    hipLaunchKernelGGL(grid_sort_scan_kernel, dim3(256), b, 0, s, counts, n_runs, totals);
    hipLaunchKernelGGL(grid_sort_scatter_kernel, sort_grid, b, 0, s, static_cast<const uint8_t*>(keys), (uint32_t)n_chain,
                       n_runs, static_cast<const uint32_t*>(counts), static_cast<const uint32_t*>(totals), perm);
    BkArgs o = a;
    o.order = perm;
    bk_chain(o, L, s, ptr.accum, (double)n_chain);
  } else {
    bk_chain(a, L, s, ptr.accum, (double)n_chain);
  }
  hipLaunchKernelGGL(bk_grid_spots_kernel, rows, b, 0, s, a, n_row, n_dates,
                     static_cast<const double*>(var_rows), spot_rows);
  return (int)hipGetLastError();
}

}
// ... 1 lines not shown
```

hedgehog.jl_amd/csrc/hh_ctx.h:

```cpp
#pragma once
#include <chrono>
#include <cstdarg>
#include <cstdio>
#include <cstring>
#include <mutex>

#include "hh_kernels.h"

struct hh_ctx {
  int device = 0;
  hipStream_t own_stream = nullptr;
  hipStream_t stream = nullptr;
  hipEvent_t ev0 = nullptr, ev1 = nullptr, ev_switch = nullptr;
  hipEvent_t ev_stage = nullptr;
  bool staged_host = false;
  double* records = nullptr;
  size_t records_cap = 0;
  uint64_t* seeds = nullptr;
  size_t seeds_cap = 0;
  double* replay = nullptr;
  size_t replay_cap = 0;
  double* replay_src = nullptr;
  size_t replay_src_cap = 0;
  double* terminal = nullptr;
  size_t terminal_cap = 0;
  double* terminal_d = nullptr;
  size_t terminal_d_cap = 0;
  double* payoffs = nullptr;
  size_t payoffs_cap = 0;
  double* basket_records = nullptr;
  size_t basket_records_cap = 0;
  double* basket_accum = nullptr;
  size_t basket_accum_cap = 0;
  unsigned char* bk_scratch = nullptr;
  size_t bk_scratch_cap = 0;
  hh::BkTableKey bk_table_key{};
  double* lsm_grid = nullptr;
  size_t lsm_grid_cap = 0;
  double* heston_var = nullptr;
  size_t heston_var_cap = 0;
  double* lsm_val = nullptr;
  size_t lsm_val_cap = 0;
  int32_t* lsm_tau = nullptr;
  size_t lsm_tau_cap = 0;
  double* lsm_scratch = nullptr;
  size_t lsm_scratch_cap = 0;
  struct {
    bool active = false;
    hh_model m{};
    uint64_t ntot = 0;
    uint32_t n_steps = 0;
    int32_t degree = 0;
    double step_discount = 1.0;
  } shard;
  int lsm_form = hh::kLsmFormAuto;
  int bk_term_cache = 0;
  uint64_t bk_last_n = 0;
  int bk_last_cache = 0;
  int grid_form = HH_GRID_FORM_BATCHED;
  int grid_order = 1;
  unsigned char* bk_sort = nullptr;
  size_t bk_sort_cap = 0;
  uint64_t lsm_persistent_fallbacks = 0;
  long long lsm_spin_ticks = -1;
  double* frecords = nullptr;
  size_t frecords_cap = 0;
  int fuse_reduce = 2;
  unsigned int* finish_state = nullptr;
  long long finish_spin_ticks = -1;
  int finish_tile_first = 0;
  struct SeedEntry {
    uint64_t* dev = nullptr;
    uint64_t n = 0, fingerprint = 0, head = 0, tail = 0, stamp = 0;
  };
  static constexpr int kSeedEntries = HH_SEED_CACHE_ENTRIES;
  SeedEntry seed_cache[kSeedEntries];
  uint64_t seed_clock = 0, seed_hits = 0, seed_uploads = 0, seed_evictions = 0;
  double* accum = nullptr;
  double* accum_host = nullptr;
  static constexpr int kTimingSlots = 256;
  bool timing = false;
  hipEvent_t tev[kTimingSlots][2] = {};
  int t_count = 0;
  char err[512] = {0};
  std::recursive_mutex mu;
};

namespace {

[[maybe_unused]] int fail(hh_ctx* ctx, int code, const char* fmt, ...) {
  if (ctx) {
    va_list ap;
    va_start(ap, fmt);
    vsnprintf(ctx->err, sizeof(ctx->err), fmt, ap);
    va_end(ap);
  }
  return code;
}

#define HH_HIP(ctx, expr)                                                                   \
  do {                                                                                      \
    hipError_t e__ = (hipError_t)(expr);                                                    \
    if (e__ != hipSuccess)                                                                  \
      return fail(ctx, HH_ERR_HIP, "%s failed: %s (%s:%d)", #expr, hipGetErrorString(e__),  \
                  __FILE__, __LINE__);                                                      \
  } while (0)

template <class T>
int ensure(hh_ctx* ctx, T*& buf, size_t& cap, size_t need) {
  if (need <= cap) return HH_OK;
  if (buf) HH_HIP(ctx, hipFree(buf));
  buf = nullptr;
  cap = 0;
  hipError_t e = hipMalloc((void**)&buf, need * sizeof(T));
  if (e != hipSuccess)
    return fail(ctx, HH_ERR_NOMEM, "hipMalloc(%zu bytes) failed: %s", need * sizeof(T),
                hipGetErrorString(e));
  cap = need;
  return HH_OK;
}

[[maybe_unused]] inline int note_host_copy(hh_ctx* ctx) {
  HH_HIP(ctx, hipEventRecord(ctx->ev_stage, ctx->stream));
  ctx->staged_host = true;
  return HH_OK;
}
template <class T>
int stage_host(hh_ctx* ctx, T*& buf, size_t& cap, size_t need, const T* src, size_t n, const T** dev) {
  int rc = ensure(ctx, buf, cap, need);
  if (rc) return rc;
  HH_HIP(ctx, hipMemcpyAsync(buf, src, n * sizeof(T), hipMemcpyHostToDevice, ctx->stream));
  if ((rc = note_host_copy(ctx))) return rc;
  *dev = buf;
  return HH_OK;
}
[[maybe_unused]] inline int release_host_operands(hh_ctx* ctx) {
  if (!ctx->staged_host) return HH_OK;
  ctx->staged_host = false;
  HH_HIP(ctx, hipEventSynchronize(ctx->ev_stage));
  return HH_OK;
}

[[maybe_unused]] inline int ensure_bk_scratch(hh_ctx* ctx, size_t need) {
  const size_t before = ctx->bk_scratch_cap;
  const int rc = ensure(ctx, ctx->bk_scratch, ctx->bk_scratch_cap, need);
  if (ctx->bk_scratch_cap != before) ctx->bk_table_key = hh::BkTableKey{};
  return rc;
}

struct WallClock {
  std::chrono::steady_clock::time_point t0 = std::chrono::steady_clock::now();
  double ms() const { return std::chrono::duration<double, std::milli>(std::chrono::steady_clock::now() - t0).count(); }
};

[[maybe_unused]] int finalize_results(const hh_model* models, size_t model_stride, const hh_config* c,
                                      const double* acc, uint32_t k, double kernel_ms, double total_ms,
                                      hh_result* out) {
  for (uint32_t i = 0; i < k; ++i) {
    std::memset(&out[i], 0, sizeof(hh_result));
    const int rc = hh_mc_finalize(&models[i * model_stride], c, acc + (size_t)i * HH_ACC_LEN, &out[i]);
    if (rc) return rc;
    out[i].kernel_ms = kernel_ms;
    out[i].total_ms = total_ms;
  }
  return HH_OK;
}

}
```

hedgehog.jl_amd/csrc/hh_kernels.h:

```cpp
#pragma once
#include <hip/hip_runtime.h>
#include <stdint.h>

#include "../../include/hedgehog_mc.h"

namespace hh {

constexpr int kTile = HH_TILE_PATHS;
constexpr int kRecStride = HH_ACC_LEN;
constexpr unsigned long long kPoison = 0x7FF8C0DE7FF8C0DEull;
constexpr unsigned long long kFinishSpinTicksDefault = 500000000ull;
constexpr int kRecItmS = 11;

template <int P>
struct DualT {
  double v;
  double d[P > 0 ? P : 1];
};

constexpr int kMaxBasis = 4;
enum { kBasisV0 = 0, kBasisKappa = 1, kBasisTheta = 2, kBasisSigma = 3 };
struct PartialMap {
  int sim;
  int n;
  int n_active;
  int basis[kMaxBasis];
  double w[HH_MAX_PARTIALS][kMaxBasis];
  double xdT[HH_MAX_PARTIALS];
  double dK[HH_MAX_PARTIALS];
};
template <int P>
struct SimArgs {
  DualT<P> x0;
  DualT<P> v0;
  DualT<P> kappa, theta, sigma;
  DualT<P> r;
  DualT<P> gdrift;
  DualT<P> strike;
  DualT<P> law_mu, law_sd;
  double dt, sqrt_dt, rho, rho_c, cp;
  uint64_t n_paths;
  uint64_t path_offset;
  uint32_t n_steps;
  uint32_t n_tiles;
  uint32_t tail_from;
  const uint64_t* seeds;
  const double* replay;
  double* terminal;
  double* terminal_d;
  double* records;
  double* accum;
  double acc_n_paths;
  unsigned int* finish_state;
  unsigned long long finish_spin_ticks;
  uint32_t reducer_tile;
  PartialMap map;
};

struct DevicePtrs {
  const uint64_t* seeds;
  const double* replay;
  double* terminal;
  double* terminal_d;
  double* records;
  double* accum;
  unsigned int* finish_state;
  long long finish_spin_ticks = -1;
  int finish_tile_first = 0;
  void* bk_scratch;
  struct BkTableKey* bk_table_key;
  int bk_term_cache;
  void* bk_sort;
  bool replay_path_major;
};
inline bool replay_direct_path_major(uint32_t n_steps, int ncomp) { return ((uint64_t)n_steps * ncomp) % 2 == 0; }
struct BkTableKey {
  const void* where;
  double nu;
  double kappa, sigma2, T;
};

constexpr int kBasketChunk = 4096;
struct BasketArgs {
  const double* terminal;
  const double* terminal_d;
  const double* strikes;
  const double* cps;
  uint64_t n_paths;
  uint32_t n_chunks;
  int antithetic;
  double* records;
};
inline uint32_t basket_chunks(uint64_t n_paths) {
  return (uint32_t)((n_paths + kBasketChunk - 1) / kBasketChunk);
}

inline uint32_t tiles_for(uint64_t n_paths) { return (uint32_t)((n_paths + kTile - 1) / kTile); }
constexpr int kExactPairs = 8, kExactPairsHuge = 64;
constexpr int kExactPairsSmall = 4;
int exact_pairs_per_lane(uint64_t n_paths);
inline uint32_t exact_records(uint64_t n_paths) {
  const uint64_t per = 512ull * (uint64_t)exact_pairs_per_lane(n_paths);
  return (uint32_t)((n_paths + per - 1) / per);
}
inline uint32_t sim_records(const hh_config& c) {
  return c.strategy == HH_EXACT_LAW ? exact_records(c.n_paths) : tiles_for(c.n_paths);
}
inline int pad_partials(uint32_t p) { return p <= 4 ? (int)p : 4; }

int launch_simulation(const hh_model& m, const hh_config& c, const DevicePtrs& p, hipStream_t s);
int launch_simulation_multi(const hh_model* models, int n_models, const hh_config& c, const DevicePtrs* p,
                            hipStream_t s);
constexpr int kMaxModelsPerPass = 4;
SimArgs<0> make_args0(const hh_model& m, const hh_config& c, const DevicePtrs& p);
struct BkTransition {
  const double* in_spot;
  const double* in_var;
  double* out_spot;
  double* out_var;
  uint32_t step;
};
bool bk_same_chain(const hh_model& a, const hh_model& b);
int launch_bk_refinish(const hh_model& m, const hh_config& c, const DevicePtrs& p, const double* rec0, hipStream_t s);
int launch_bk(const hh_model& m, const hh_config& c, const DevicePtrs& p, hipStream_t s,
              const BkTransition* tr = nullptr, bool upload_tables = true);
int launch_bk_grid(const hh_model& m, const hh_config& c, const DevicePtrs& p, hipStream_t s,
                   double* spot_rows, double* var_rows, uint32_t k0, uint32_t n_dates, bool upload_tables);
uint32_t bk_grid_dates_per_chain(uint64_t n_paths, uint32_t n_steps, int term_cache);
size_t bk_grid_sort_bytes(uint64_t n_chain);
constexpr int kBkTermCacheDefault = 256;
size_t bk_scratch_bytes(uint64_t n_paths, int term_cache = 0);
void bk_diag_ptrs(const void* scratch, uint64_t n_paths, int term_cache, const uint32_t** decisions,
                  const uint32_t** series_len);
uint32_t bk_record_count(uint64_t n_paths);
const uint32_t* bk_live_records(const void* scratch, uint64_t n_paths);
int launch_copy_bk_counters(const double* src, double* accum, uint32_t n_groups, hipStream_t s);
int launch_fill_rows(double* spot0, double* var0, uint64_t n, double S0, double V0, hipStream_t s);
int launch_reduce_records(const double* records, uint32_t n_records, double n_paths, double* accum,
                          hipStream_t s, uint32_t n_groups = 1, const hh_model* m = nullptr,
                          const hh_config* c = nullptr, bool basket = false,
                          const uint32_t* n_records_dev = nullptr);
int count_active_partials(const hh_model& m, const hh_config& c);
int launch_basket_payoffs(const BasketArgs& b, uint32_t n_payoffs, uint32_t n_active_partials,
                          hipStream_t s);
int launch_carr_madan(const hh_model& m, int dynamics, int compat_sqrt_alpha, double alpha,
                      double bound, double* out_dev, hipStream_t s);
int launch_carr_madan_grad(const hh_model& m, int dynamics, int compat_sqrt_alpha, double alpha,
                           double bound, const double* per_payoff_dev, uint32_t n_payoffs,
                           double* out_dev, hipStream_t s);
int launch_carr_madan_basket(const hh_model& m, int dynamics, int compat_sqrt_alpha, double alpha,
                             double bound, const double* per_payoff_dev, uint32_t n_payoffs,
                             double* out_dev, hipStream_t s);
struct CrrTree {
  double F, K, cp, u, p, q, disc;
  int32_t style;
  uint32_t row;
};
int launch_crr(const CrrTree* trees_dev, const double* spot_factors_dev, int steps, uint32_t n_trees,
               double* out_dev, hipStream_t s);
uint32_t lsm_chunks(uint64_t ntot);
size_t lsm_scratch_doubles(uint64_t ntot, uint32_t n_steps, int degree);
enum { kLsmPhaseStats = 0, kLsmPhasePow = 1, kLsmPhaseInit = 2, kLsmPhaseStep = 3, kLsmPhaseFinal = 4 };
int launch_lsm_phase(int phase, uint32_t t, const double* grid, uint64_t ntot, uint32_t n_steps,
                     double strike, double cp, double step_discount, int degree, int32_t* tau,
                     double* val, double* scratch, double* records, const double* vec_in,
                     double* vec_out, hipStream_t s);
int launch_gbm_grid(const uint64_t* seeds_dev, uint64_t n_paths, uint32_t n_steps, double S0,
                    double r, double sigma, double T, int anti, double* grid, hipStream_t s);
int launch_euler_grid(const hh_model& m, const hh_config& c, const uint64_t* seeds_dev, bool log_state,
                      double* grid, double* var_grid, hipStream_t s);
enum { kLsmFormPerDate = 0, kLsmFormPersistent = 1, kLsmFormAuto = 2 };
int launch_lsm(const double* grid, uint64_t ntot, uint32_t n_steps, double strike, double cp,
               double step_discount, int degree, int32_t* tau, double* val, double* scratch,
               double* records, hipStream_t s, int form, int* form_used,
               unsigned long long spin_ticks = 100000000ull );
const unsigned int* lsm_persistent_status(const double* scratch);
constexpr int kLsmStampSlotsApi = 8;
int launch_wiener_fill(int dynamics, double rho, double sqrt_dt, uint32_t n_steps, uint64_t n_paths,
                       const uint64_t* seeds_dev, double* dst, hipStream_t s);
int launch_replay_pack(int ncomp, uint64_t n_paths, uint32_t n_steps, const double* src_dev,
                       double* dst_dev, hipStream_t s);

}
```

hedgehog.jl_amd/csrc/hh_kernels.hip:

```cpp
#include <type_traits>

#include "hh_sim.h"

namespace hh {



constexpr int kReplayChunk = 4;
constexpr int kReplayMaxWaves = 2;
constexpr int kReplayMaxWavesDual = 3;
constexpr int kReplayMaxWavesAnti = 8;

constexpr int replay_max_waves(bool replay, bool anti, int p) {
  return !replay ? 8 : anti ? kReplayMaxWavesAnti : p > 0 ? kReplayMaxWavesDual : kReplayMaxWaves;
}
template <class M, int P, bool REPLAY, bool ANTI>
__global__ __launch_bounds__(kTile)
__attribute__((amdgpu_waves_per_eu(1, replay_max_waves(REPLAY, ANTI, P)))) void euler_kernel(const SimArgs<P> a) {
  constexpr int NC = M::NCOMP;
  using State = typename M::State;

  const uint32_t tile = blockIdx.x;
  const uint32_t tid = threadIdx.x;
  const uint64_t path = (uint64_t)tile * kTile + tid;
// ... 188 lines not shown
      if constexpr (ANTI) M::step(sa, a, -d.x, -d.y);
    } else {
      M::step(st, a, d.x, 0.0);
      if constexpr (ANTI) M::step(sa, a, -d.x, 0.0);
      M::step(st, a, d.y, 0.0);
      if constexpr (ANTI) M::step(sa, a, -d.y, 0.0);
    }
  };

  if (n_chunks > 0) issue(0, true);
  for (int k = 0; k < n_chunks; ++k) {
    V2 d[NP];
#pragma unroll
    for (int j = 0; j < NP; ++j)
      d[j] = *reinterpret_cast<const V2*>(my_img + (((uint32_t)j ^ sw) << 4));
    asm volatile("s_waitcnt lgkmcnt(0)" ::: "memory");
    __builtin_amdgcn_sched_barrier(0);
    const bool full = k >= 1 && k <= k_full_end;
    if (k + 1 < n_chunks) issue(k + 1, !(k + 1 <= k_full_end));
    if (full) {
#pragma unroll
      for (int j = 0; j < NP; ++j) advance(d[j]);
    } else {
#pragma unroll
      for (int j = 0; j < NP; ++j) {
        const int t = NP * k - o + j;
        if (t >= 0 && t < T) advance(d[j]);
      }
    }
  }

  double acc[4 + P];
#pragma unroll
  for (int i = 0; i < 4 + P; ++i) acc[i] = 0.0;
  finish_path<P, ANTI>(st, sa, a, path, acc);
  block_reduce_publish<4 + P, kTile / 64, 2>(acc, a.records + (size_t)tile * kRecStride, a.accum != nullptr, a.map.n > 0);
  if (a.accum && reduces_records(tile, a)) finish_records<kTile, P>(a);
}


template <int P>
struct ExactState {
  DualT<P> x;
};

template <int P, bool REPLAY, bool ANTI, int PAIRS>
__global__ __launch_bounds__(kTile) void exact_gbm_kernel(const SimArgs<P> a) {
  const uint32_t chunk = blockIdx.x;
  const uint32_t tid = threadIdx.x;

  double acc[4 + P];
#pragma unroll
  for (int i = 0; i < 4 + P; ++i) acc[i] = 0.0;

#pragma unroll 2
  for (int jp = 0; jp < PAIRS; ++jp) {
    const uint64_t path0 = ((uint64_t)chunk * PAIRS + jp) * (2 * kTile) + (uint64_t)tid * 2;
    double z[2];
    exact_pair_normals<REPLAY>(a, path0, z);
#pragma unroll
    for (int j = 0; j < 2; ++j) {
      ExactState<P> st, sa;
      st.x.v = fma(a.law_sd.v, z[j], a.law_mu.v);
      if constexpr (ANTI) sa.x.v = 2 * a.law_mu.v - st.x.v;
      if constexpr (P > 0) {
#pragma unroll
        for (int k = 0; k < P; ++k) {
          st.x.d[k] = fma(a.law_sd.d[k], z[j], a.law_mu.d[k]);
          if constexpr (ANTI) sa.x.d[k] = 2 * a.law_mu.d[k] - st.x.d[k];
        }
      }
      finish_path<P, ANTI>(st, sa, a, path0 + j, acc);
    }
  }
  block_reduce_publish<4 + P, kTile / 64, 2>(acc, a.records + (size_t)chunk * kRecStride, a.accum != nullptr, a.map.n > 0);
  if (a.accum && reduces_records(chunk, a)) finish_records<kTile, P>(a);
}


__global__ __launch_bounds__(256) void reduce_records_kernel(const double* __restrict__ rec,
                                                              uint32_t n, double n_paths,
                                                              double* __restrict__ accum,
                                                              const PartialMap map,
                                                              const uint32_t* __restrict__ n_dev) {
  __shared__ double sm[257];
  const int slot = blockIdx.x;
  rec += (size_t)blockIdx.y * n * kRecStride;
  if (n_dev) n = min(n, *n_dev);
  accum += (size_t)blockIdx.y * kRecStride;
  double out;
  const int k = slot - HH_ACC_DSUM;
  if (map.n > 0 && k >= 0 && k < HH_MAX_PARTIALS) {
    out = 0.0;
    if (k < map.n) {
      for (int j = 0; j < map.n_active; ++j)
        if (map.w[k][j] != 0.0) out = fma(map.w[k][j], sum_slot(rec, n, HH_ACC_DSUM + j, sm), out);
      if (map.xdT[k] != 0.0) out = fma(map.xdT[k], sum_slot(rec, n, kRecItmS, sm), out);
      if (map.dK[k] != 0.0) out -= map.dK[k] * sum_slot(rec, n, kRecItmS + 1, sm);
    }
  } else if (map.sim && (slot == kRecItmS || slot == kRecItmS + 1)) {
    out = 0.0;
  } else {
    out = sum_slot(rec, n, slot, sm);
  }
  if (threadIdx.x == 0) accum[slot] = (slot == HH_ACC_NPATHS) ? n_paths : out;
}


constexpr int kFillSteps = 16;

template <int NC>
__global__ __launch_bounds__(kTile) void wiener_fill_kernel(double rho, double rho_c,
                                                            double sqrt_dt, uint32_t n_steps,
                                                            uint64_t n_paths,
                                                            const uint64_t* __restrict__ seeds,
                                                            double* __restrict__ dst) {
  const uint32_t tile = blockIdx.x;
  const uint32_t s0 = blockIdx.y * kFillSteps;
  const uint64_t path = (uint64_t)tile * kTile + threadIdx.x;
  const bool live = path < n_paths;
  const uint64_t key = live ? seeds[path] : 0ull;
  double* out = dst + (size_t)tile * n_steps * NC * kTile + threadIdx.x;
  for (uint32_t s = s0; s < s0 + kFillSteps && s < n_steps; ++s) {
    double z1, z2;
    if constexpr (NC == 2) {
      normal_pair(key, s, 0u, 0u, kDomEuler, z1, z2);
      const double d1 = sqrt_dt * z1;
      const double d2 = sqrt_dt * fma(rho, z1, rho_c * z2);
      out[((size_t)s * 2 + 0) * kTile] = live ? d1 : 0.0;
      out[((size_t)s * 2 + 1) * kTile] = live ? d2 : 0.0;
    } else {
      normal_pair(key, s >> 1, 0u, 0u, kDomEuler, z1, z2);
      const double d = sqrt_dt * ((s & 1u) ? z2 : z1);
      out[(size_t)s * kTile] = live ? d : 0.0;
    }
  }
}

constexpr int kPackSteps = 4;

template <int NC>
__global__ __launch_bounds__(256) void replay_pack_kernel(uint64_t n_paths, uint32_t n_steps,
                                                          const double* __restrict__ src,
                                                          double* __restrict__ dst) {
  constexpr int COLS = kPackSteps * NC;
  __shared__ double sm[kTile][COLS + 1];
  const uint32_t tile = blockIdx.x;
  const uint32_t s0 = blockIdx.y * kPackSteps;
  const int tid = threadIdx.x;
  const int col = tid % COLS, row0 = tid / COLS;
  constexpr int ROWS_PER_IT = 256 / COLS;
  for (int row = row0; row < kTile; row += ROWS_PER_IT) {
    const uint64_t path = (uint64_t)tile * kTile + row;
    const uint32_t s = s0 + col / NC;
    double v = 0.0;
    if (path < n_paths && s < n_steps) v = src[((size_t)path * n_steps + s0) * NC + col];
    sm[row][col] = v;
  }
  __syncthreads();
  double* out = dst + (size_t)tile * n_steps * NC * kTile + tid;
  for (int c = 0; c < COLS; ++c) {
    const uint32_t s = s0 + c / NC;
    if (s < n_steps) out[((size_t)s * NC + (c % NC)) * kTile] = sm[tid][c];
  }
}


static inline double seed_of(const double* p, uint32_t k, uint32_t n) {
  return (p && k < n) ? p[k] : 0.0;
}

static const double* basis_seeds(const hh_model& m, int b) {
  return b == kBasisV0 ? m.dV0 : b == kBasisKappa ? m.dkappa : b == kBasisTheta ? m.dtheta : m.dsigma;
}

static PartialMap classify_partials(const hh_model& m, const hh_config& c) {
  PartialMap pm{};
  const uint32_t np = c.n_partials < HH_MAX_PARTIALS ? c.n_partials : HH_MAX_PARTIALS;
  pm.n = (int)np;
  const bool euler = c.strategy == HH_EULER_MARUYAMA;
  const bool heston = c.dynamics == HH_HESTON;
  const double dt = m.T / (double)(c.n_steps ? c.n_steps : 1);
  const double sqT = sqrt(m.T), tmul = c.compat_sqrt_alpha ? sqT : m.T;
  for (int b = 0; b < kMaxBasis; ++b) {
    if (b != kBasisSigma && !(heston && euler)) continue;
    bool used = false;
    for (uint32_t k = 0; k < np; ++k) used = used || seed_of(basis_seeds(m, b), k, np) != 0.0;
    if (used) pm.basis[pm.n_active++] = b;
  }
  for (uint32_t k = 0; k < np; ++k) {
    for (int j = 0; j < pm.n_active; ++j) pm.w[k][j] = seed_of(basis_seeds(m, pm.basis[j]), k, np);
    pm.dK[k] = seed_of(m.dstrike, k, np);
    const double dr = seed_of(m.dr_drift, k, np);
    double xd = seed_of(m.dS0, k, np) / m.S0;
    if (euler) {
      if (dr != 0.0)
        for (uint32_t s = 0; s < c.n_steps; ++s) xd = fma(dt, dr, xd);
    } else {
      xd = xd + dr * tmul;
    }
    pm.xdT[k] = xd;
  }
  return pm;
}

int exact_pairs_per_lane(uint64_t n_paths) {
  return n_paths >= (uint64_t)2048 * 512 * kExactPairsHuge ? kExactPairsHuge
         : n_paths >= (uint64_t)2048 * 512 * kExactPairs   ? kExactPairs
                                                           : kExactPairsSmall;
}

int count_active_partials(const hh_model& m, const hh_config& c) {
  return classify_partials(m, c).n_active;
}

template <int P>
static SimArgs<P> make_args(const hh_model& m, const hh_config& c, const DevicePtrs& p,
                            const PartialMap& pm) {
  SimArgs<P> a{};
  const double sig2h = 0.5 * m.sigma * m.sigma;
  a.x0.v = log(m.S0);
  a.v0.v = m.V0;
  a.kappa.v = m.kappa;
  a.theta.v = m.theta;
  a.sigma.v = m.sigma;
  a.r.v = m.r_drift;
  a.gdrift.v = m.r_drift - sig2h;
  a.strike.v = m.strike;
  const double sqT = sqrt(m.T);
  const double tmul = c.compat_sqrt_alpha ? sqT : m.T;
  a.law_mu.v = a.x0.v + a.gdrift.v * tmul;
  a.law_sd.v = m.sigma * sqT;
  for (int j = 0; j < P && j < pm.n_active; ++j) {
    const int b = pm.basis[j];
    const double dsig = b == kBasisSigma ? 1.0 : 0.0;
    a.v0.d[j] = b == kBasisV0 ? 1.0 : 0.0;
    a.kappa.d[j] = b == kBasisKappa ? 1.0 : 0.0;
    a.theta.d[j] = b == kBasisTheta ? 1.0 : 0.0;
    a.sigma.d[j] = dsig;
    a.gdrift.d[j] = -m.sigma * dsig;
    a.law_mu.d[j] = a.gdrift.d[j] * tmul;
    a.law_sd.d[j] = dsig * sqT;
  }
  a.dt = m.T / (double)(c.n_steps ? c.n_steps : 1);
  a.sqrt_dt = sqrt(a.dt);
  a.rho = m.rho;
  a.rho_c = sqrt(1.0 - m.rho * m.rho);
  a.cp = m.cp;
  a.n_paths = c.n_paths;
  a.path_offset = c.path_offset;
  a.n_steps = c.n_steps;
  a.n_tiles = sim_records(c);
  a.seeds = p.seeds;
  a.replay = p.replay;
  a.terminal = p.terminal;
  a.terminal_d = p.terminal_d;
  a.records = p.records;
  a.accum = p.accum;
  a.acc_n_paths = (double)c.n_paths;
  a.finish_state = p.finish_state;
  a.finish_spin_ticks = p.finish_spin_ticks < 0 ? kFinishSpinTicksDefault : (unsigned long long)p.finish_spin_ticks;
  a.reducer_tile = p.finish_tile_first ? 0u : a.n_tiles - 1u;
  a.map = pm;
  return a;
}

SimArgs<0> make_args0(const hh_model& m, const hh_config& c, const DevicePtrs& p) {
  hh_config c0 = c;
  c0.n_partials = 0;
  return make_args<0>(m, c0, p, classify_partials(m, c0));
}

template <class M, int P, bool REPLAY, bool ANTI>
static int launch_euler_t(const SimArgs<P>& a, hipStream_t s) {
  hipLaunchKernelGGL((euler_kernel<M, P, REPLAY, ANTI>), dim3(a.n_tiles), dim3(kTile), 0, s, a);
  return (int)hipGetLastError();
}

template <class M, int P>
static int launch_euler_pm(const SimArgs<P>& a, bool anti, hipStream_t s) {
  auto kernel = anti ? euler_pm_kernel<M, P, true> : euler_pm_kernel<M, P, false>;
  hipLaunchKernelGGL(kernel, dim3(a.n_tiles), dim3(kTile), 0, s, a);
  return (int)hipGetLastError();
}

template <class M, int P>
static int launch_euler_m(const SimArgs<P>& a, bool replay, bool anti, hipStream_t s, bool path_major = false) {
  if (replay && path_major) return launch_euler_pm<M, P>(a, anti, s);
  if (replay) return anti ? launch_euler_t<M, P, true, true>(a, s) : launch_euler_t<M, P, true, false>(a, s);
  return anti ? launch_euler_t<M, P, false, true>(a, s) : launch_euler_t<M, P, false, false>(a, s);
}

template <int P>
static int launch_sim_p(const hh_model& m, const hh_config& c, const DevicePtrs& p,
                        const PartialMap& pm, hipStream_t s) {
  const SimArgs<P> a = make_args<P>(m, c, p, pm);
  const bool anti = c.antithetic != 0;
  const bool replay = c.noise_mode == HH_NOISE_REPLAY;
  if (c.strategy == HH_EXACT_LAW) {
    auto pick = [&](auto replay_c, auto anti_c) {
      constexpr bool R = decltype(replay_c)::value, A = decltype(anti_c)::value;
      const int pairs = exact_pairs_per_lane(c.n_paths);
      return pairs == kExactPairsHuge ? exact_gbm_kernel<P, R, A, kExactPairsHuge>
             : pairs == kExactPairs   ? exact_gbm_kernel<P, R, A, kExactPairs>
             : pairs == 4             ? exact_gbm_kernel<P, R, A, 4>
             : pairs == 2             ? exact_gbm_kernel<P, R, A, 2>
                                      : exact_gbm_kernel<P, R, A, 1>;
    };
    using T = std::true_type;
    using F = std::false_type;
    auto kernel = replay ? (anti ? pick(T{}, T{}) : pick(T{}, F{})) : (anti ? pick(F{}, T{}) : pick(F{}, F{}));
    hipLaunchKernelGGL(kernel, dim3(a.n_tiles), dim3(kTile), 0, s, a);
    return (int)hipGetLastError();
  }
  const bool direct = replay && p.replay_path_major;
  if (c.dynamics == HH_LOGNORMAL) return launch_euler_m<GbmModel<P>, P>(a, replay, anti, s, direct);
  if (c.em_split) return launch_euler_m<HestonModel<P, true>, P>(a, replay, anti, s, direct);
  return launch_euler_m<HestonModel<P, false>, P>(a, replay, anti, s, direct);
}

int launch_simulation(const hh_model& m, const hh_config& c, const DevicePtrs& p, hipStream_t s) {
  const PartialMap pm = classify_partials(m, c);
  switch (pad_partials((uint32_t)pm.n_active)) {
    case 0: return launch_sim_p<0>(m, c, p, pm, s);
    case 1: return launch_sim_p<1>(m, c, p, pm, s);
    case 2: return launch_sim_p<2>(m, c, p, pm, s);
    case 3: return launch_sim_p<3>(m, c, p, pm, s);
    default: return launch_sim_p<4>(m, c, p, pm, s);
  }
}

int launch_reduce_records(const double* records, uint32_t n_records, double n_paths, double* accum,
                          hipStream_t s, uint32_t n_groups, const hh_model* m, const hh_config* c,
                          bool basket, const uint32_t* n_records_dev) {
  PartialMap pm{};
  if (m && c && (basket || c->strategy != HH_BROADIE_KAYA)) {
    if (c->n_partials) pm = classify_partials(*m, *c);
    pm.sim = 1;
    if (basket)
      for (double& d : pm.dK) d = 0.0;
  }
  hipLaunchKernelGGL(reduce_records_kernel, dim3(kRecStride, n_groups), dim3(256), 0, s, records,
                     n_records, n_paths, accum, pm, n_records_dev);
  return (int)hipGetLastError();
}


constexpr int kBasketKB = 4;

template <int P>
__global__ __launch_bounds__(256) void basket_payoff_kernel(const BasketArgs b, const uint32_t n_payoffs) {
  const uint32_t per_xcd = (b.n_chunks + 7u) / 8u;
  const uint32_t xcd = blockIdx.x & 7u, idx = blockIdx.x >> 3;
  const uint32_t grp = idx / per_xcd, chunk = (idx % per_xcd) * 8u + xcd;
  if (chunk >= b.n_chunks) return;
  const uint32_t k0 = grp * kBasketKB;
  double strike[kBasketKB], cp[kBasketKB];
#pragma unroll
  for (int g = 0; g < kBasketKB; ++g) {
    const uint32_t k = min(k0 + g, n_payoffs - 1);
    strike[g] = b.strikes[k];
    cp[g] = b.cps[k];
  }
  const uint64_t n_total = b.antithetic ? 2 * b.n_paths : b.n_paths;
  double acc[kBasketKB][4 + P];
#pragma unroll
  for (int g = 0; g < kBasketKB; ++g)
#pragma unroll
    for (int i = 0; i < 4 + P; ++i) acc[g][i] = 0.0;
  const uint64_t i0 = (uint64_t)chunk * kBasketChunk;
  for (uint32_t j = threadIdx.x; j < (uint32_t)kBasketChunk; j += 256) {
    const uint64_t i = i0 + j;
    if (i >= b.n_paths) break;
    const double S = b.terminal[i];
    double Sa = 0.0, d[P > 0 ? P : 1], da[P > 0 ? P : 1];
    if constexpr (P > 0) {
#pragma unroll
      for (int q = 0; q < P; ++q) d[q] = b.terminal_d[(uint64_t)q * n_total + i];
    }
    if (b.antithetic) {
      Sa = b.terminal[b.n_paths + i];
      if constexpr (P > 0) {
#pragma unroll
        for (int q = 0; q < P; ++q) da[q] = b.terminal_d[(uint64_t)q * n_total + b.n_paths + i];
      }
    }
#pragma unroll
    for (int g = 0; g < kBasketKB; ++g) {
      const double m = cp[g] * (S - strike[g]);
      const bool itm = m > 0.0;
      double p = itm ? m : 0.0;
      double wS = itm ? cp[g] * S : 0.0, wN = itm ? cp[g] : 0.0;
      double pd[P > 0 ? P : 1];
      if constexpr (P > 0) {
#pragma unroll
        for (int q = 0; q < P; ++q) pd[q] = itm ? cp[g] * d[q] : 0.0;
      }
      if (b.antithetic) {
        const double ma = cp[g] * (Sa - strike[g]);
        const bool itma = ma > 0.0;
        p = (p + (itma ? ma : 0.0)) / 2;
        wS = (wS + (itma ? cp[g] * Sa : 0.0)) / 2;
        wN = (wN + (itma ? cp[g] : 0.0)) / 2;
        if constexpr (P > 0) {
#pragma unroll
          for (int q = 0; q < P; ++q) pd[q] = (pd[q] + (itma ? cp[g] * da[q] : 0.0)) / 2;
        }
      }
      acc[g][0] += p;
      acc[g][1] = fma(p, p, acc[g][1]);
      if constexpr (P > 0) {
#pragma unroll
        for (int q = 0; q < P; ++q) acc[g][2 + q] += pd[q];
      }
      acc[g][2 + P] += wS;
      acc[g][3 + P] += wN;
    }
  }
#pragma unroll
  for (int g = 0; g < kBasketKB; ++g) {
    if (k0 + g >= n_payoffs) break;
    if (g) __syncthreads();
    block_reduce_store<4 + P, 4, 2>(acc[g], b.records + ((size_t)(k0 + g) * b.n_chunks + chunk) * kRecStride);
  }
}

// ... 56 lines not shown
```

hedgehog.jl_amd/csrc/hh_mgpu.hip:

```cpp
#include <dlfcn.h>

#include <array>
#include <atomic>
#include <chrono>
#include <condition_variable>
#include <cstdlib>
#include <cstring>
#include <functional>
#include <memory>
#include <thread>
#include <vector>

#include "hh_ctx.h"

namespace {

typedef struct ncclComm* rccl_comm_t;
constexpr int kNcclSuccess = 0, kNcclSum = 0, kNcclDouble = 8;

struct RcclApi {
  void* lib = nullptr;
  int (*CommInitAll)(rccl_comm_t*, int, const int*) = nullptr;
  int (*CommDestroy)(rccl_comm_t) = nullptr;
  int (*CommAbort)(rccl_comm_t) = nullptr;
// ... 183 lines not shown
  mg->workers.clear();
}

int for_each_device(hh_mgpu* mg, const std::function<int(int)>& fn) {
  for (int g = 0; g < mg->n; ++g) mg->derr[g][0] = 0;
  bool threads = mg->enqueue == HH_MGPU_ENQUEUE_THREADS && mg->n > 1;
  if (threads && mg->workers.empty()) {
    mg->workers.resize(mg->n - 1);
    for (int g = 1; g < mg->n && threads; ++g) {
      mg->workers[g - 1].reset(new (std::nothrow) hh_worker());
      if (!mg->workers[g - 1]) {
        threads = false;
        break;
      }
      try {
        mg->workers[g - 1]->th = std::thread(worker_main, mg, g);
      } catch (...) {
        threads = false;
      }
    }
    if (!threads) {
      stop_workers(mg);
      mg->enqueue = HH_MGPU_ENQUEUE_SERIAL;
    }
  }
  if (!threads) {
    for (int g = 0; g < mg->n; ++g) mg->rcs[g] = fn(g);
  } else {
    mg->job = &fn;
    for (int g = 1; g < mg->n; ++g) {
      hh_worker& w = *mg->workers[g - 1];
      w.posted.fetch_add(1);
      if (w.parked.load()) {
        std::lock_guard<std::mutex> lk(w.m);
        w.cv.notify_one();
      }
    }
    mg->rcs[0] = fn(0);
    for (int g = 1; g < mg->n; ++g) {
      hh_worker& w = *mg->workers[g - 1];
      const uint64_t want = w.posted.load();
      const auto t0 = clk::now();
      while (w.finished.load() != want) {
        if (us_since(t0) < 2000.0) cpu_relax(); else std::this_thread::yield();
      }
      mg->rcs[g] = w.rc;
    }
    mg->job = nullptr;
  }
  for (int g = 0; g < mg->n; ++g)
    if (mg->rcs[g]) return mfail(mg, mg->rcs[g], "shard %d (device %d): %s", g, mg->devices[g], mg->derr[g].data());
  return HH_OK;
}


int ensure_acc(hh_mgpu* mg, size_t n_acc) {
  for (int g = 0; g < mg->n; ++g) {
    if (mg->acc_cap[g] >= n_acc) continue;
    HH_MHIP(mg, hipSetDevice(mg->devices[g]));
    if (mg->acc[g]) HH_MHIP(mg, hipFree(mg->acc[g]));
    if (mg->red[g]) HH_MHIP(mg, hipFree(mg->red[g]));
    mg->acc[g] = mg->red[g] = nullptr;
    mg->acc_cap[g] = 0;
    if (hipMalloc((void**)&mg->acc[g], n_acc * sizeof(double)) != hipSuccess ||
        hipMalloc((void**)&mg->red[g], n_acc * sizeof(double)) != hipSuccess)
      return mfail(mg, HH_ERR_NOMEM, "hipMalloc of the accumulator vectors failed");
    mg->acc_cap[g] = n_acc;
  }
  if (mg->host_cap < n_acc * (size_t)mg->n) {
    if (mg->host) HH_MHIP(mg, hipHostFree(mg->host));
    mg->host = nullptr;
    mg->host_cap = 0;
    HH_MHIP(mg, hipHostMalloc((void**)&mg->host, n_acc * (size_t)mg->n * sizeof(double), hipHostMallocDefault));
    mg->host_cap = n_acc * (size_t)mg->n;
  }
  return HH_OK;
}

int drain(hh_mgpu* mg, int rc) {
  for (int g = 0; g < mg->n; ++g) {
    (void)hipSetDevice(mg->devices[g]);
    (void)hipStreamSynchronize(mg->ctx[g]->stream);
    mg->ctx[g]->shard.active = false;
  }
  return rc;
}
#define HH_MHIP_DRAIN(mg, expr)                                                                       \
  do {                                                                                                \
    hipError_t e__ = (hipError_t)(expr);                                                              \
    if (e__ != hipSuccess)                                                                            \
      return drain(mg, mfail(mg, HH_ERR_HIP, "%s failed: %s (%s:%d)", #expr, hipGetErrorString(e__), \
                             __FILE__, __LINE__));                                                    \
  } while (0)


int all_reduce_group(hh_mgpu* mg, double* const* send, double* const* recv, size_t n) {
  RcclApi& api = rccl();
  int e = api.GroupStart();
  for (int g = 0; g < mg->n && e == kNcclSuccess; ++g)
    e = api.AllReduce(send[g], recv[g], n, kNcclDouble, kNcclSum, mg->comms[g], mg->ctx[g]->stream);
  const int e2 = api.GroupEnd();
  return e == kNcclSuccess ? e2 : e;
}

bool rccl_give_up(hh_mgpu* mg) {
  RcclApi& api = rccl();
  for (rccl_comm_t c : mg->comms)
    if (c) (void)api.CommAbort(c);
  mg->comms.clear();
  mg->mode = HH_MGPU_REDUCE_HOST;
  mg->rccl_lost = true;
  bool all_moved = true;
  for (int g = 0; g < mg->n; ++g) {
    hh_ctx* c = mg->ctx[g];
    std::lock_guard<std::recursive_mutex> lock__(c->mu);
    c->shard.active = false;
    hipStream_t fresh = nullptr;
    (void)hipSetDevice(mg->devices[g]);
    if (c->stream != c->own_stream || hipStreamCreateWithFlags(&fresh, hipStreamNonBlocking) != hipSuccess) {
      all_moved = false;
      continue;
    }
    if (mg->fence[g]) (void)hipStreamWaitEvent(fresh, mg->fence[g], 0);
    mg->retired.push_back({mg->devices[g], c->own_stream});
    c->own_stream = c->stream = fresh;
  }
  mg->stuck = mg->stuck || !all_moved;
  return all_moved;
}

void wait_fences(hh_mgpu* mg) {
  for (int g = 0; g < mg->n; ++g)
    if (mg->fence[g]) {
      (void)hipSetDevice(mg->devices[g]);
      (void)hipEventSynchronize(mg->fence[g]);
    }
}

struct Basket {
  const double *strikes, *cps;
  uint32_t n_payoffs;
  uint32_t n_models = 0;
};

int run_shards(hh_mgpu* mg, const hh_model* m, const hh_config* cfgs, const Basket* basket,
               double* const* terminals, double* kernel_ms) {
  const bool multi = basket && basket->n_models > 0;
  const size_t n_acc = (size_t)HH_ACC_LEN * (multi ? basket->n_models : basket ? basket->n_payoffs : 1u);
  if (mg->stuck)
    return mfail(mg, HH_ERR_RCCL, "a collective failed and a shard could not be moved off the stream it was enqueued on "
                                  "(a stream lent with hh_ctx_set_stream, or no new stream): create a new context");
  if (mg->flags == HH_MGPU_RCCL && mg->rccl_lost)
    return drain(mg, mfail(mg, HH_ERR_RCCL, "the RCCL communicators of this context were aborted after a failed "
                                            "collective (HH_MGPU_RCCL does not fall back): create a new one"));
  int rc = ensure_acc(mg, n_acc);
  if (rc) return drain(mg, rc);
  const auto t_enq = clk::now();
  rc = for_each_device(mg, [&](int g) -> int {
    const auto t0 = clk::now();
    hh_ctx* c = mg->ctx[g];
    HH_DHIP(mg, g, hipSetDevice(mg->devices[g]));
    HH_DHIP(mg, g, hipEventRecord(c->ev0, c->stream));
    if (cfgs[g].n_paths == 0) {
      HH_DHIP(mg, g, hipMemsetAsync(mg->acc[g], 0, n_acc * sizeof(double), c->stream));
    } else {
      double* term = terminals ? terminals[g] : nullptr;
      const int r = multi    ? hh_mc_accumulate_multi(c, m, basket->n_models, &cfgs[g], mg->acc[g], nullptr)
                    : basket ? hh_mc_accumulate_basket(c, m, &cfgs[g], basket->strikes, basket->cps,
                                                       basket->n_payoffs, mg->acc[g], term)
                             : hh_mc_accumulate(c, m, &cfgs[g], mg->acc[g], term);
      if (r) {
        snprintf(mg->derr[g].data(), mg->derr[g].size(), "%s", hh_last_error(c));
        return r;
      }
    }
    HH_DHIP(mg, g, hipEventRecord(c->ev1, c->stream));
    mg->fence[g] = c->ev1;
    mg->enq_us[g] = us_since(t0);
    return HH_OK;
  });
  mg->enq_phase_us = us_since(t_enq);
  if (rc) return drain(mg, rc);
  bool reduced = false;
  if (mg->mode == HH_MGPU_REDUCE_RCCL) {
    const int e = all_reduce_group(mg, mg->acc.data(), mg->red.data(), n_acc);
    if (e == kNcclSuccess) {
      HH_MHIP_DRAIN(mg, hipSetDevice(mg->devices[0]));
      HH_MHIP_DRAIN(mg, hipMemcpyAsync(mg->host, mg->red[0], n_acc * sizeof(double), hipMemcpyDeviceToHost,
                                       mg->ctx[0]->stream));
      reduced = true;
    } else {
      mfail(mg, HH_ERR_RCCL, "ncclAllReduce failed: %s — communicators aborted, accumulators are summed on the host",
            rccl().GetErrorString(e));
      const bool moved = rccl_give_up(mg);
      if (mg->flags == HH_MGPU_RCCL || !moved) {
        wait_fences(mg);
        return HH_ERR_RCCL;
      }
    }
  }
  if (!reduced) {
    for (int g = 0; g < mg->n; ++g) {
      HH_MHIP_DRAIN(mg, hipSetDevice(mg->devices[g]));
      HH_MHIP_DRAIN(mg, hipMemcpyAsync(mg->host + (size_t)g * n_acc, mg->acc[g], n_acc * sizeof(double),
                                       hipMemcpyDeviceToHost, mg->ctx[g]->stream));
    }
  }
  for (int g = 0; g < mg->n; ++g) {
    HH_MHIP_DRAIN(mg, hipSetDevice(mg->devices[g]));
    HH_MHIP_DRAIN(mg, hipStreamSynchronize(mg->ctx[g]->stream));
  }
  if (!reduced) {
    for (int g = 1; g < mg->n; ++g)
      for (size_t i = 0; i < n_acc; ++i) mg->host[i] += mg->host[(size_t)g * n_acc + i];
  }
  double worst = 0.0;
  for (int g = 0; g < mg->n; ++g) {
    float ms = 0.f;
    HH_MHIP(mg, hipSetDevice(mg->devices[g]));
    HH_MHIP(mg, hipEventElapsedTime(&ms, mg->ctx[g]->ev0, mg->ctx[g]->ev1));
    if (ms > worst) worst = ms;
  }
  *kernel_ms = worst;
  return HH_OK;
}

int ncomp(int dynamics) { return dynamics == HH_HESTON ? 2 : 1; }

}

extern "C" {

void hh_mgpu_shard_range(uint64_t n_paths, int n_devices, int g, int tile_aligned, uint64_t* start,
                         uint64_t* stop) {
  uint64_t a = 0, b = 0;
  if (n_devices > 0 && g >= 0 && g < n_devices) shard_range(n_paths, n_devices, g, tile_aligned != 0, &a, &b);
  if (start) *start = a;
  if (stop) *stop = b;
}

int hh_mgpu_create(hh_mgpu** out, const int* device_ids, int n_devices, int flags) {
  if (!out) return HH_ERR_INVALID;
  *out = nullptr;
  if (!device_ids || n_devices < 1 || n_devices > 64) return HH_ERR_INVALID;
  if (flags != HH_MGPU_AUTO && flags != HH_MGPU_HOST_SUM && flags != HH_MGPU_RCCL) return HH_ERR_INVALID;
  int n_hip = 0;
  if (hipGetDeviceCount(&n_hip) != hipSuccess || n_hip <= 0) return HH_ERR_HIP;
  for (int g = 0; g < n_devices; ++g)
    if (device_ids[g] < 0 || device_ids[g] >= n_hip) return HH_ERR_INVALID;
  hh_mgpu* mg = new (std::nothrow) hh_mgpu();
  if (!mg) return HH_ERR_NOMEM;
  mg->n = n_devices;
  mg->flags = flags;
  mg->devices.assign(device_ids, device_ids + n_devices);
  mg->ctx.assign(n_devices, nullptr);
  mg->acc.assign(n_devices, nullptr);
  mg->red.assign(n_devices, nullptr);
  mg->acc_cap.assign(n_devices, 0);
  mg->xchg.assign(n_devices, nullptr);
  mg->xchg_cap.assign(n_devices, 0);
  mg->rcs.assign(n_devices, 0);
  mg->derr.resize(n_devices);
  mg->enq_us.assign(n_devices, 0.0);
  mg->pre.assign(n_devices, nullptr);
  mg->fence.assign(n_devices, nullptr);
  for (int g = 0; g < n_devices; ++g) {
    int rc = hh_ctx_create(&mg->ctx[g], device_ids[g]);
    if (!rc && hipEventCreateWithFlags(&mg->pre[g], hipEventDisableTiming) != hipSuccess) rc = HH_ERR_HIP;
    if (rc) {
      hh_mgpu_destroy(mg);
      return rc;
    }
  }
  const bool want = flags == HH_MGPU_RCCL || (flags == HH_MGPU_AUTO && n_devices > 1);
  if (want) {
    RcclApi& api = rccl();
    int e = -1;
    if (api.ok) {
      mg->comms.assign(n_devices, nullptr);
      e = api.CommInitAll(mg->comms.data(), n_devices, device_ids);
      if (e != kNcclSuccess) {
        mg->comms.clear();
        mfail(mg, HH_ERR_RCCL, "ncclCommInitAll failed: %s — accumulators are summed on the host",
              api.GetErrorString(e));
      }
    } else {
      mfail(mg, HH_ERR_RCCL, "RCCL unavailable: %s — accumulators are summed on the host", api.why);
    }
    if (e == kNcclSuccess) {
      mg->mode = HH_MGPU_REDUCE_RCCL;
    } else if (flags == HH_MGPU_RCCL) {
      hh_mgpu_destroy(mg);
      return HH_ERR_RCCL;
    }
  }
// ... 475 lines not shown
```

hedgehog.jl_amd/csrc/hh_sim.h:

```cpp
#pragma once
#include <type_traits>

#include "hh_kernels.h"
#include "hh_reduce.h"
#include "hh_rng.h"

namespace hh {


__device__ __forceinline__ double sqrt_clipped(double w) {
  const double y = __builtin_fmin(__builtin_amdgcn_rsq(w), 0x1p1000);
  double g = w * y, h = 0.5 * y;
  const double r = fma(-h, g, 0.5);
  g = fma(g, r, g);
  h = fma(h, r, h);
  g = fma(fma(-g, g, w), h, g);
  return fma(fma(-g, g, w), h, g);
}

template <int P, bool SPLIT>
struct HestonModel {
  static constexpr int NCOMP = 2;
  struct State {
    DualT<P> x, v;
// ... 123 lines not shown
                                            uint64_t path, double (&acc)[4 + P]) {
  if (path >= a.n_paths) return;
  double S, p, pd[P > 0 ? P : 1], wS, wN;
  payoff_of<P>(st.x, a, S, p, pd, wS, wN);
  if (a.terminal) a.terminal[path] = S;
  const uint64_t n_total = ANTI ? 2 * a.n_paths : a.n_paths;
  if constexpr (P > 0) {
    if (a.terminal_d) {
#pragma unroll
      for (int k = 0; k < P; ++k) a.terminal_d[(uint64_t)k * n_total + path] = S * st.x.d[k];
    }
  }
  if constexpr (ANTI) {
    double Sa, pa, pda[P > 0 ? P : 1], wSa, wNa;
    payoff_of<P>(sa.x, a, Sa, pa, pda, wSa, wNa);
    if (a.terminal) a.terminal[a.n_paths + path] = Sa;
    if constexpr (P > 0) {
      if (a.terminal_d) {
#pragma unroll
        for (int k = 0; k < P; ++k)
          a.terminal_d[(uint64_t)k * n_total + a.n_paths + path] = Sa * sa.x.d[k];
      }
    }
    p = (p + pa) / 2;
    wS = (wS + wSa) / 2;
    wN = (wN + wNa) / 2;
    if constexpr (P > 0) {
#pragma unroll
      for (int k = 0; k < P; ++k) pd[k] = (pd[k] + pda[k]) / 2;
    }
  }
  acc[0] += p;
  acc[1] = fma(p, p, acc[1]);
  if constexpr (P > 0) {
#pragma unroll
    for (int k = 0; k < P; ++k) acc[2 + k] += pd[k];
  }
  acc[2 + P] += wS;
  acc[3 + P] += wN;
}

template <bool REPLAY, int P>
__device__ __forceinline__ void exact_pair_normals(const SimArgs<P>& a, uint64_t path0, double (&z)[2]) {
  if constexpr (REPLAY) {
    z[0] = path0 < a.n_paths ? a.replay[path0] : 0.0;
    z[1] = path0 + 1 < a.n_paths ? a.replay[path0 + 1] : 0.0;
  } else {
    const uint64_t g0 = a.path_offset + path0;
    const uint64_t key = a.seeds[0];
    double z1, z2;
    normal_pair(key, (uint32_t)(g0 >> 1), (uint32_t)(g0 >> 33), 0u, kDomExactGbm, z1, z2);
    if ((g0 & 1ull) == 0) {
      z[0] = z1;
      z[1] = z2;
    } else {
      z[0] = z2;
      const uint64_t g1 = g0 + 1;
      normal_pair(key, (uint32_t)(g1 >> 1), (uint32_t)(g1 >> 33), 0u, kDomExactGbm, z1, z2);
      z[1] = z1;
    }
  }
}


template <class Args>
__device__ __forceinline__ bool reduces_records(uint32_t tile, const Args& a) {
  return tile == a.reducer_tile;
}
__device__ __forceinline__ unsigned int scalar_load_begin(const unsigned int* p) {
  unsigned int v;
  asm volatile("s_load_dword %0, %1, 0x0" : "=s"(v) : "s"(p) : "memory");
  return v;
}
__device__ __forceinline__ unsigned int scalar_load_end(unsigned int v) {
  asm volatile("s_waitcnt lgkmcnt(0)" : "+s"(v) : : "memory");
  return v;
}

__device__ __forceinline__ void store_through(double* p, double v) {
  __hip_atomic_store(p, v, __ATOMIC_RELAXED, __HIP_MEMORY_SCOPE_AGENT);
}
__device__ __forceinline__ double load_through(const double* p) {
  return __hip_atomic_load(p, __ATOMIC_RELAXED, __HIP_MEMORY_SCOPE_AGENT);
}
__device__ __forceinline__ bool is_poison(double v) {
  return (unsigned long long)__double_as_longlong(v) == kPoison;
}
__device__ __forceinline__ double publish_value(double v) {
  return is_poison(v) ? __longlong_as_double((long long)(kPoison ^ 1ull)) : v;
}

template <int N, int NWAVES, int TAIL>
__device__ __forceinline__ void block_reduce_publish(double (&acc)[N], double* __restrict__ rec, bool publish,
                                                     bool itm_live) {
#pragma unroll
  for (int i = 0; i < N; ++i) {
#pragma unroll
    for (int off = 32; off > 0; off >>= 1) acc[i] += __shfl_down(acc[i], off, 64);
  }
  __shared__ double sm[NWAVES][N];
  const int lane = threadIdx.x & 63, wave = threadIdx.x >> 6;
  if (lane == 0) {
#pragma unroll
    for (int i = 0; i < N; ++i) sm[wave][i] = acc[i];
  }
  __syncthreads();
  if (threadIdx.x < (unsigned)kRecStride) {
    const int slot = threadIdx.x;
    static_assert(N - TAIL <= kRecItmS, "payoff sums and in-the-money sums overlap");
    const int i = slot < N - TAIL ? slot
                  : (slot >= kRecItmS && slot < kRecItmS + TAIL) ? N - TAIL + (slot - kRecItmS) : -1;
    double t = 0.0;
    if (i >= 0) {
      t = sm[0][i];
#pragma unroll
      for (int w = 1; w < NWAVES; ++w) t += sm[w][i];
    }
    if (!publish) rec[slot] = t;
    else if (i >= 0 && (slot < kRecItmS || itm_live)) store_through(rec + slot, publish_value(t));
  }
}

constexpr int kFinishBatch = 16;
using u32x4 = __attribute__((__vector_size__(4 * sizeof(unsigned int)))) unsigned int;

__device__ __forceinline__ bool keep_waiting(unsigned long long& t0, bool& give, unsigned int* gave_up,
                                             unsigned long long spin_ticks, const unsigned int* state) {
  const unsigned long long now = wall_clock64();
  if (t0 == 0) t0 = now;
  if (now - t0 >= spin_ticks) {
    *gave_up = 1u;
    give = true;
    return false;
  }
  if (now - t0 > 2000ull && __hip_atomic_load(state, __ATOMIC_RELAXED, __HIP_MEMORY_SCOPE_AGENT) != 0u) {
    give = true;
    return false;
  }
  __builtin_amdgcn_s_sleep(8);
  return true;
}

template <int NT>
__device__ __forceinline__ void partial_pairs(const double* rec, uint32_t n, double* __restrict__ sm,
                                              unsigned int* gave_up, unsigned long long spin_ticks, const unsigned int* state) {
  static_assert(256 % NT == 0, "the 256 virtual threads are dealt evenly");
  const auto rsrc = __builtin_amdgcn_make_buffer_rsrc(const_cast<double*>(rec), 0, (int)(n * (uint32_t)(kRecStride * 8)), 0x00020000);
  bool give = *gave_up != 0u;
  for (int vt = threadIdx.x; vt < 256; vt += NT) {
    double t0 = 0.0, t1 = 0.0;
    for (uint32_t b = vt; b < n; b += 256 * kFinishBatch) {
      u32x4 v[kFinishBatch];
      unsigned long long since = 0;
      for (;;) {
        bool there = true;
#pragma unroll
        for (int u = 0; u < kFinishBatch; ++u) {
          const uint32_t i = b + 256u * u;
          v[u] = u32x4{0u, 0u, 0u, 0u};
          if (i < n) v[u] = __builtin_amdgcn_raw_buffer_load_b128(rsrc, (int)(i * (uint32_t)(kRecStride * 8)), 0, 16);
          const unsigned long long lo = ((unsigned long long)v[u][1] << 32) | v[u][0];
          const unsigned long long hi = ((unsigned long long)v[u][3] << 32) | v[u][2];
          there = there && lo != kPoison && hi != kPoison;
        }
        if (there || give || !keep_waiting(since, give, gave_up, spin_ticks, state)) break;
      }
// ... 29 lines not shown
#pragma unroll
          for (int q = 0; q < NS; ++q) {
            v[q][u] = i < n ? load_through(rec + (size_t)i * kRecStride + slot_of(q)) : 0.0;
            there = there && !is_poison(v[q][u]);
          }
        }
        if (there || give || !keep_waiting(since, give, gave_up, spin_ticks, state)) break;
      }
#pragma unroll
      for (int q = 0; q < NS; ++q)
#pragma unroll
        for (int u = 0; u < kB; ++u) t[q] += v[q][u];
    }
#pragma unroll
    for (int q = 0; q < NS; ++q) sm[q * 256 + vt] = t[q];
  }
}

template <int NT, int P, class Args>
__device__ __forceinline__ void finish_records(const Args& a) {
  double* __restrict__ records = a.records;
  double* __restrict__ accum = a.accum;
  const uint32_t n_rec = a.n_tiles;
  const double n_paths = a.acc_n_paths;
  const PartialMap* map = &a.map;
  const unsigned long long spin_ticks = a.finish_spin_ticks;
  __shared__ double sm[4 * 256];
  __shared__ unsigned int gave_up;
  const unsigned int state_in_flight = scalar_load_begin(a.finish_state);
  if (threadIdx.x == 0) gave_up = 0u;
  __syncthreads();
  const bool itm = map->n > 0;
  const double poison = __longlong_as_double((long long)kPoison);
  const auto wsrc = __builtin_amdgcn_make_buffer_rsrc(records, 0, (int)(n_rec * (uint32_t)(kRecStride * 8)), 0x00020000);
  const unsigned int ph = (unsigned int)(kPoison >> 32), pl = (unsigned int)kPoison;
  partial_pairs<NT>(records, n_rec, sm, &gave_up, spin_ticks, a.finish_state);
  if (itm) partial_slots<NT, 2>(records, n_rec, [](int q) { return kRecItmS + q; }, sm + 512, &gave_up, spin_ticks, a.finish_state);
  for (uint32_t i = threadIdx.x; i < n_rec; i += NT) {
    __builtin_amdgcn_raw_buffer_store_b128(u32x4{pl, ph, pl, ph}, wsrc, (int)(i * (uint32_t)(kRecStride * 8)), 0, 16);
    if (itm) {
      store_through(records + (size_t)i * kRecStride + kRecItmS, poison);
      store_through(records + (size_t)i * kRecStride + kRecItmS + 1, poison);
    }
  }
  __syncthreads();
  double s[4] = {0.0, 0.0, 0.0, 0.0}, d[P > 0 ? P : 1];
  if (threadIdx.x < 64) {
    s[0] = tree256(sm);
    s[1] = tree256(sm + 256);
    if (itm) {
      s[2] = tree256(sm + 512);
      s[3] = tree256(sm + 768);
    }
  }
  if constexpr (P > 0) {
    __syncthreads();
    partial_slots<NT, P>(records, n_rec, [](int q) { return HH_ACC_DSUM + q; }, sm, &gave_up, spin_ticks, a.finish_state);
    for (uint32_t i = threadIdx.x; i < n_rec; i += NT) {
#pragma unroll
      for (int j = 0; j < P; ++j) store_through(records + (size_t)i * kRecStride + HH_ACC_DSUM + j, poison);
    }
    __syncthreads();
    if (threadIdx.x < 64) {
#pragma unroll
      for (int j = 0; j < P; ++j) d[j] = tree256(sm + j * 256);
    }
  }
  if (threadIdx.x < (unsigned)kRecStride) {
    const int slot = threadIdx.x;
    double out = slot == HH_ACC_SUM ? s[0] : slot == HH_ACC_SUMSQ ? s[1] : 0.0;
    const int k = slot - HH_ACC_DSUM;
    if (k >= 0 && k < map->n) {
      out = 0.0;
      if constexpr (P > 0) {
#pragma unroll
        for (int j = 0; j < P; ++j)
          if (j < map->n_active && map->w[k][j] != 0.0) out = fma(map->w[k][j], d[j], out);
      }
      if (map->xdT[k] != 0.0) out = fma(map->xdT[k], s[2], out);
      if (map->dK[k] != 0.0) out -= map->dK[k] * s[3];
    }
    if (slot == HH_ACC_NPATHS) out = n_paths;
    const bool dirty = scalar_load_end(state_in_flight) != 0u;
    accum[slot] = (gave_up || dirty) ? __longlong_as_double(0x7FF8000000000000ll) : out;
    if (slot == 0 && gave_up) __hip_atomic_store(a.finish_state, 1u, __ATOMIC_RELAXED, __HIP_MEMORY_SCOPE_AGENT);
  }
}


__device__ __forceinline__ double stream_load(const double* p) { return __builtin_nontemporal_load(p); }

}
```

include/hedgehog_mc.h:

```cpp
#ifndef HEDGEHOG_MC_H
#define HEDGEHOG_MC_H

#include <stddef.h>
#include <stdint.h>

#ifdef __cplusplus
extern "C" {
#endif

#define HH_ABI_VERSION 6
#define HH_MAX_PARTIALS 8
#define HH_TILE_PATHS 256
#define HH_ACC_LEN 16
#define HH_MAX_MODELS 16

#define HH_ACC_SUM 0
#define HH_ACC_SUMSQ 1
#define HH_ACC_DSUM 2
#define HH_ACC_NPATHS 10
#define HH_ACC_BK_NEWTON_FAIL 11
#define HH_ACC_BK_BISECT 12
#define HH_ACC_BK_MAXGUESS 13
#define HH_ACC_BK_CF_TERMS 14

enum hh_status {
  HH_OK = 0,
  HH_ERR_INVALID = -1,
  HH_ERR_UNSUPPORTED = -2,
  HH_ERR_HIP = -3,
  HH_ERR_NOMEM = -4,
  HH_ERR_RCCL = -5,
  HH_ERR_DEVICE_TIMEOUT = -6
};

enum hh_dynamics { HH_LOGNORMAL = 0, HH_HESTON = 1 };
enum hh_strategy { HH_EULER_MARUYAMA = 0, HH_EXACT_LAW = 1, HH_BROADIE_KAYA = 2 };
enum hh_noise_mode { HH_NOISE_GENERATE = 0, HH_NOISE_REPLAY = 1 };
enum hh_replay_layout { HH_REPLAY_TILE_MAJOR = 0, HH_REPLAY_PATH_MAJOR = 1 };

enum hh_bk_root_form { HH_BK_ROOT_SECANT = 0,
                       HH_BK_ROOT_ORDER2 = 1 };
enum hh_bk_bracket_form { HH_BK_BRACKET_MIDPOINT = 0,
                          HH_BK_BRACKET_ROOTS = 1 };
enum hh_bk_caps { HH_BK_CAPS_AS_WRITTEN = 0,
                  HH_BK_CAPS_ROOTS_DEFAULT = 1 };

typedef struct hh_ctx hh_ctx;

typedef struct hh_model {
  double S0, V0, kappa, theta, sigma, rho;
  double r_drift, discount, T, strike, cp;
  const double *dS0, *dV0, *dkappa, *dtheta, *dsigma, *dr_drift, *ddiscount, *dstrike;
} hh_model;

typedef struct hh_config {
  int32_t dynamics;
  int32_t strategy;
  int32_t antithetic;
  int32_t em_split;
  int32_t compat_sqrt_alpha;
  int32_t noise_mode;
  int32_t replay_layout;
  int32_t seeds_on_device;
  int32_t replay_on_device;
  int32_t terminal_on_device;
  uint32_t n_steps;
  uint32_t n_partials;
  uint64_t n_paths;
  uint64_t path_offset;
  const uint64_t* seeds;
  const double* replay;
  double bk_n_sigma;
  double bk_cf_tol;
  double bk_atol;
  double bk_moment_h;
  int32_t bk_newton_maxiter;
  int32_t bk_bisect_maxiter;
  int32_t bk_root_form;
  int32_t bk_bracket_form;
  int32_t bk_caps;
  int32_t reserved0;
  uint64_t seeds_len;
  uint64_t replay_len;
} hh_config;

typedef struct hh_result {
  double price;
  double std_error;
  double sum_payoff, sumsq_payoff;
  double dprice[HH_MAX_PARTIALS];
  uint64_t n_paths_done;
  uint64_t bk_newton_fail, bk_bisect_fallback, bk_maxguess_fallback, bk_cf_terms;
  double kernel_ms;
  double total_ms;
} hh_result;

int hh_abi_version(void);

int hh_ctx_create(hh_ctx** out, int device_id);
void hh_ctx_destroy(hh_ctx* ctx);
int hh_ctx_set_stream(hh_ctx* ctx, void* hip_stream);
int hh_ctx_reset_stream(hh_ctx* ctx);
const char* hh_last_error(const hh_ctx* ctx);
enum hh_option { HH_OPT_LSM_FORM = 1, HH_OPT_BK_TERM_CACHE = 2, HH_OPT_GRID_FORM = 3, HH_OPT_LSM_SPIN_TICKS = 4,
                 HH_OPT_FUSE_REDUCE = 5, HH_OPT_GRID_ORDER = 6, HH_OPT_FINISH_SPIN_TICKS = 7,
                 HH_OPT_FINISH_TILE_FIRST = 8 };
enum hh_grid_form { HH_GRID_FORM_PER_DATE = 0, HH_GRID_FORM_BATCHED = 1 };
enum hh_lsm_form { HH_LSM_FORM_PER_DATE = 0, HH_LSM_FORM_PERSISTENT = 1, HH_LSM_FORM_AUTO = 2 };
int hh_ctx_set_option(hh_ctx* ctx, int32_t option, int64_t value);
int hh_ctx_check_last(hh_ctx* ctx);

int hh_mc_solve(hh_ctx* ctx, const hh_model* model, const hh_config* cfg, hh_result* out,
                double* terminal);

int hh_mc_accumulate(hh_ctx* ctx, const hh_model* model, const hh_config* cfg, double* accum_dev,
                     double* terminal);
int hh_mc_finalize(const hh_model* model, const hh_config* cfg, const double* accum_host,
                   hh_result* out);

int hh_mc_solve_multi(hh_ctx* ctx, const hh_model* models, uint32_t n_models, const hh_config* cfg,
                      hh_result* out, double* const* terminals);
int hh_mc_accumulate_multi(hh_ctx* ctx, const hh_model* models, uint32_t n_models, const hh_config* cfg,
                           double* accum_dev, double* const* terminals);

int hh_bk_decisions(hh_ctx* ctx, uint64_t n_paths, uint32_t* decisions, uint32_t* series_len);

typedef struct hh_mgpu hh_mgpu;
enum hh_mgpu_flags { HH_MGPU_AUTO = 0, HH_MGPU_HOST_SUM = 1, HH_MGPU_RCCL = 2 };
enum hh_mgpu_reduce { HH_MGPU_REDUCE_HOST = 0, HH_MGPU_REDUCE_RCCL = 1 };
int hh_mgpu_create(hh_mgpu** out, const int* device_ids, int n_devices, int flags);
void hh_mgpu_destroy(hh_mgpu* mg);
const char* hh_mgpu_last_error(const hh_mgpu* mg);
int hh_mgpu_n_devices(const hh_mgpu* mg);
int hh_mgpu_reduce_mode(const hh_mgpu* mg);
int hh_mgpu_selftest(hh_mgpu* mg, int32_t* ranks_out, int32_t* reduce_mode_out );
int hh_mgpu_rccl_info(const hh_mgpu* mg, char* path_out, size_t cap, int32_t* version_out, int32_t* from_env_out);
enum hh_mgpu_option { HH_MGPU_OPT_ENQUEUE = 1 };
enum hh_mgpu_enqueue { HH_MGPU_ENQUEUE_SERIAL = 0, HH_MGPU_ENQUEUE_THREADS = 1  };
int hh_mgpu_set_option(hh_mgpu* mg, int32_t option, int64_t value);
int hh_mgpu_enqueue_stats(hh_mgpu* mg, double* shard_us, double* phase_us);
hh_ctx* hh_mgpu_ctx(hh_mgpu* mg, int i);
void hh_mgpu_shard_range(uint64_t n_paths, int n_devices, int g, int tile_aligned, uint64_t* start,
                         uint64_t* stop);
int hh_mgpu_solve(hh_mgpu* mg, const hh_model* model, const hh_config* cfg, hh_result* out,
                  double* terminal);
int hh_mgpu_solve_shards(hh_mgpu* mg, const hh_model* model, const hh_config* shard_cfgs ,
                         hh_result* out, double* const* terminals );
int hh_mgpu_solve_basket(hh_mgpu* mg, const hh_model* model, const hh_config* cfg, const double* strikes,
                         const double* cps, uint32_t n_payoffs, hh_result* out );
int hh_mgpu_solve_multi(hh_mgpu* mg, const hh_model* models, uint32_t n_models, const hh_config* cfg,
                        hh_result* out );


int hh_mc_accumulate_basket(hh_ctx* ctx, const hh_model* model, const hh_config* cfg,
                            const double* strikes, const double* cps, uint32_t n_payoffs,
                            double* accum_dev, double* terminal);
int hh_mc_solve_basket(hh_ctx* ctx, const hh_model* model, const hh_config* cfg,
                       const double* strikes, const double* cps, uint32_t n_payoffs,
                       hh_result* out , double* terminal);

int hh_carr_madan(hh_ctx* ctx, const hh_model* model, int32_t dynamics, int32_t compat_sqrt_alpha,
                  double alpha, double bound, double* price_out);
int hh_carr_madan_basket(hh_ctx* ctx, const hh_model* model, int32_t dynamics,
                         int32_t compat_sqrt_alpha, double alpha, double bound, const double* strikes,
                         const double* cps, const double* Ts, const double* r_drifts,
                         const double* discounts, uint32_t n_payoffs, double* prices_out);
enum hh_cm_grad { HH_CM_GRAD_S0 = 0, HH_CM_GRAD_V0, HH_CM_GRAD_KAPPA, HH_CM_GRAD_THETA, HH_CM_GRAD_SIGMA,
                  HH_CM_GRAD_RHO, HH_CM_GRAD_R_DRIFT, HH_CM_GRAD_DISCOUNT, HH_CM_GRAD_LEN };
int hh_carr_madan_basket_grad(hh_ctx* ctx, const hh_model* model, int32_t dynamics,
                              int32_t compat_sqrt_alpha, double alpha, double bound,
                              const double* strikes, const double* cps, const double* Ts,
                              const double* r_drifts, const double* discounts, uint32_t n_payoffs,
                              double* prices_out, double* grad_out);

#define HH_CRR_MAX_STEPS 32768
#define HH_CRR_FORM_A_MAX_STEPS 2047
enum hh_crr_style { HH_CRR_EUROPEAN = 0, HH_CRR_AMERICAN_FORWARD = 1, HH_CRR_AMERICAN_SPOT = 2 };
int hh_crr_solve(hh_ctx* ctx, int32_t steps, uint32_t n_trees, const double* forwards, const double* strikes,
                 const double* cps, const double* ups, const double* discounts, const int32_t* styles,
                 const double* spot_factors, uint32_t n_spot_rows, const uint32_t* spot_row_of_tree,
                 double* prices_out);

typedef struct hh_lsm_result {
  double price, std_error;
  uint64_t n_paths_total;
  uint32_t rows_regressed, rows_skipped;
  double kernel_ms, total_ms;
  int32_t form;
  int32_t persistent_fallbacks;
// ... 60 lines not shown
```

Baseline: 438.4 billion.

## Deliver reduced sums directly into mapped host memory and spin-poll for arrival

The reducing workgroup now also writes its final sums with system-scope stores into a pinned, mapped, coherent host buffer. The host poisons that buffer before launch and spin-polls it for arrival instead of issuing a device-to-host copy and a stream synchronize, with event-query fallbacks and a timeout bound. The goal is to cut the completion latency of the copy and sync at the end of each solve, including multi-GPU host-sum solves. In exchange it adds host CPU busy-waiting, extra fallback paths, and relies on coherence of system-scope stores to host memory.

```diff
diff --git a/hedgehog.jl_amd/_ffi.py b/hedgehog.jl_amd/_ffi.py
--- a/hedgehog.jl_amd/_ffi.py
+++ b/hedgehog.jl_amd/_ffi.py
@@ -80,6 +80,7 @@
 HH_OPT_GRID_ORDER = 6
 HH_OPT_FINISH_SPIN_TICKS = 7
 HH_OPT_FINISH_TILE_FIRST = 8
+HH_OPT_RESULT_DELIVERY = 9
 HH_GRID_FORM_PER_DATE, HH_GRID_FORM_BATCHED = 0, 1
 HH_CM_GRAD_LEN = 8
 HH_LSM_FORM_PER_DATE, HH_LSM_FORM_PERSISTENT, HH_LSM_FORM_AUTO = 0, 1, 2
diff --git a/hedgehog.jl_amd/csrc/hh_api.hip b/hedgehog.jl_amd/csrc/hh_api.hip
--- a/hedgehog.jl_amd/csrc/hh_api.hip
+++ b/hedgehog.jl_amd/csrc/hh_api.hip
@@ -1,3 +1,4 @@
+#include <algorithm>
 #include <cmath>
 #include <cstdarg>
 #include <cstdio>
@@ -147,6 +148,46 @@
   return rf ? rf : fail(ctx, rc, "finalize failed: the accumulator holds no trajectories");
 }
 
+int ensure_mirror(hh_ctx* ctx, size_t need) {
+  if (need <= ctx->mirror_cap) return HH_OK;
+  if (ctx->mirror) {
+    HH_HIP(ctx, hipStreamSynchronize(ctx->stream));
+    HH_HIP(ctx, hipHostFree(ctx->mirror));
+  }
+  ctx->mirror = ctx->mirror_dev = nullptr;
+  ctx->mirror_cap = 0;
+  hipError_t e = hipHostMalloc((void**)&ctx->mirror, need * sizeof(double), hipHostMallocMapped | hipHostMallocCoherent);
+  if (e != hipSuccess)
+    return fail(ctx, HH_ERR_NOMEM, "hipHostMalloc(%zu bytes) failed: %s", need * sizeof(double), hipGetErrorString(e));
+  ctx->mirror_cap = need;
+  void* dev = nullptr;
+  if (hipHostGetDevicePointer(&dev, ctx->mirror, 0) == hipSuccess) ctx->mirror_dev = (double*)dev;
+  else (void)hipGetLastError();
+  return HH_OK;
+}
+
+struct Disarm {
+  hh_ctx* ctx;
+  ~Disarm() { ctx->mirror_armed = 0; }
+};
+
+inline void cpu_pause() {
+#if defined(__x86_64__)
+  __builtin_ia32_pause();
+#endif
+}
+
+inline bool all_arrived(const double* mirror, size_t n) {
+  const unsigned long long* w = reinterpret_cast<const unsigned long long*>(mirror);
+  for (size_t i = 0; i < n; ++i)
+    if (__atomic_load_n(w + i, __ATOMIC_RELAXED) == hh::kPoison) return false;
+  __atomic_thread_fence(__ATOMIC_ACQUIRE);
+  return true;
+}
+
+constexpr double kEventLookFirstUs = 200.0;
+constexpr double kEventSpinUs = 200.0;
+
 size_t replay_elems(uint64_t n_paths, uint32_t n_steps, int dynamics) {
   return (size_t)hh::tiles_for(n_paths) * n_steps * ncomp_of(dynamics) * hh::kTile;
 }
@@ -163,6 +204,96 @@
   *mean = acc[HH_ACC_SUM] / n;
   *var = n > 1.0 ? (acc[HH_ACC_SUMSQ] - n * *mean * *mean) / (n - 1.0) : 0.0;
   if (!(*var > 0.0)) *var = 0.0;
+}
+
+}
+
+namespace hh {
+
+int arm_delivery(hh_ctx* ctx, size_t n_words, bool by_copy) {
+  ctx->mirror_armed = 0;
+  const int rc = ensure_mirror(ctx, n_words);
+  if (rc) return rc;
+  if (by_copy || ctx->result_delivery != HH_RESULT_DELIVERY_MIRROR || !ctx->mirror_dev) return HH_OK;
+  unsigned long long* w = reinterpret_cast<unsigned long long*>(ctx->mirror);
+  for (size_t i = 0; i < n_words; ++i) __atomic_store_n(w + i, kPoison, __ATOMIC_RELAXED);
+  __atomic_thread_fence(__ATOMIC_RELEASE);
+  ctx->mirror_armed = n_words;
+  return HH_OK;
+}
+
+int await_delivery(hh_ctx* const* ctx, int n, double* const* dev, size_t n_words, int* bad) {
+  using clock = std::chrono::steady_clock;
+  auto us_since = [](clock::time_point t) { return std::chrono::duration<double, std::micro>(clock::now() - t).count(); };
+#define HH_HIP_G(g, expr)         \
+  do {                            \
+    if (bad) *bad = (g);          \
+    HH_HIP(ctx[g], expr);         \
+  } while (0)
+  int waiting = 0;
+  double bound_us = 0.0;
+  for (int g = 0; g < n; ++g)
+    if (ctx[g]->mirror_armed) {
+      ++waiting;
+      const long long t = ctx[g]->finish_spin_ticks < 0 ? (long long)kFinishSpinTicksDefault : ctx[g]->finish_spin_ticks;
+      bound_us = std::max(bound_us, (double)t * 0.01);
+    }
+  if (waiting) {
+    const auto t0 = clock::now();
+    double next_look = kEventLookFirstUs;
+    std::vector<char> there(n, 0);
+    for (unsigned spin = 0; waiting; ++spin) {
+      for (int g = 0; g < n; ++g)
+        if (ctx[g]->mirror_armed && !there[g] && all_arrived(ctx[g]->mirror, n_words)) {
+          there[g] = 1;
+          --waiting;
+        }
+      if (!waiting) break;
+      cpu_pause();
+      if ((spin & 31u) != 31u) continue;
+      const double t = us_since(t0);
+      if (t >= next_look) {
+        next_look = 2.0 * t;
+        for (int g = 0; g < n; ++g)
+          if (ctx[g]->mirror_armed && !there[g] && hipEventQuery(ctx[g]->ev1) == hipSuccess &&
+              !all_arrived(ctx[g]->mirror, n_words)) {
+            ctx[g]->mirror_armed = 0;
+            --waiting;
+          }
+      }
+      if (t >= bound_us)
+        for (int g = 0; g < n; ++g)
+          if (ctx[g]->mirror_armed && !there[g]) {
+            ctx[g]->mirror_armed = 0;
+            --waiting;
+          }
+    }
+  }
+  for (int g = 0; g < n; ++g)
+    if (!ctx[g]->mirror_armed) {
+      if (n > 1) HH_HIP_G(g, hipSetDevice(ctx[g]->device));
+      HH_HIP_G(g, hipMemcpyAsync(ctx[g]->mirror, dev[g], n_words * sizeof(double), hipMemcpyDeviceToHost, ctx[g]->stream));
+    }
+  for (int g = 0; g < n; ++g) {
+    if (!ctx[g]->mirror_armed) {
+      if (n > 1) HH_HIP_G(g, hipSetDevice(ctx[g]->device));
+      HH_HIP_G(g, hipStreamSynchronize(ctx[g]->stream));
+      continue;
+    }
+    ctx[g]->mirror_armed = 0;
+    const auto t1 = clock::now();
+    hipError_t e = hipEventQuery(ctx[g]->ev1);
+    while (e == hipErrorNotReady && us_since(t1) < kEventSpinUs) {
+      cpu_pause();
+      e = hipEventQuery(ctx[g]->ev1);
+    }
+    if (e != hipSuccess) {
+      (void)hipGetLastError();
+      HH_HIP_G(g, hipEventSynchronize(ctx[g]->ev1));
+    }
+  }
+#undef HH_HIP_G
+  return HH_OK;
 }
 
 }
@@ -189,7 +320,8 @@
       hipMalloc((void**)&ctx->finish_state, 2 * sizeof(unsigned int)) != hipSuccess ||
       hipMemset(ctx->finish_state, 0, 2 * sizeof(unsigned int)) != hipSuccess ||
       hipHostMalloc((void**)&ctx->accum_host, (HH_ACC_LEN + 8) * sizeof(double), hipHostMallocDefault) !=
-          hipSuccess) {
+          hipSuccess ||
+      ensure_mirror(ctx, (size_t)HH_MAX_MODELS * HH_ACC_LEN) != HH_OK) {
     hh_ctx_destroy(ctx);
     return HH_ERR_HIP;
   }
@@ -225,6 +357,7 @@
   if (ctx->frecords) (void)hipFree(ctx->frecords);
   if (ctx->finish_state) (void)hipFree(ctx->finish_state);
   if (ctx->accum_host) (void)hipHostFree(ctx->accum_host);
+  if (ctx->mirror) (void)hipHostFree(ctx->mirror);
   for (auto& pr : ctx->tev)
     for (auto& e : pr)
       if (e) (void)hipEventDestroy(e);
@@ -299,6 +432,11 @@
       if (value < 0 || value > 2)
         return fail(ctx, HH_ERR_INVALID, "HH_OPT_FUSE_REDUCE: 0 (a second kernel reduces the records), 1 (the simulation kernel does) or 2 (by size)");
       ctx->fuse_reduce = (int)value;
+      return HH_OK;
+    case HH_OPT_RESULT_DELIVERY:
+      if (value != HH_RESULT_DELIVERY_COPY && value != HH_RESULT_DELIVERY_MIRROR)
+        return fail(ctx, HH_ERR_INVALID, "HH_OPT_RESULT_DELIVERY: 0 (a copy and a wait for the stream) or 1 (the reducing workgroup stores the sums into host memory)");
+      ctx->result_delivery = (int)value;
       return HH_OK;
     default:
       return fail(ctx, HH_ERR_INVALID, "unknown option %d", option);
@@ -423,6 +561,7 @@
     p.accum = accum_dev;
     fused_controls(ctx, p);
   }
+  if (accum_dev && ctx->mirror_armed) p.accum_mirror = ctx->mirror_dev;
   if (reduced) *reduced = fuse || bk;
   if (bk) {
     rc = ensure_bk_scratch(ctx, hh::bk_scratch_bytes(c->n_paths, ctx->bk_term_cache));
@@ -492,7 +631,8 @@
   rc = run_simulation(ctx, m, c, terminal, false, nullptr, accum_dev, &reduced);
   if (rc) return rc;
   if (!reduced)
-    HH_HIP(ctx, hh::launch_reduce_records(ctx->records, hh::sim_records(*c), (double)c->n_paths, accum_dev, ctx->stream, 1, m, c));
+    HH_HIP(ctx, hh::launch_reduce_records(ctx->records, hh::sim_records(*c), (double)c->n_paths, accum_dev, ctx->stream, 1, m, c,
+                                          false, nullptr, ctx->mirror_armed ? ctx->mirror_dev : nullptr));
   if ((rc = end_timing(ctx))) return rc;
   if ((rc = release_host_operands(ctx))) return rc;
   return copy_back_terminal(ctx, c, terminal);
@@ -518,6 +658,7 @@
   if (n_models == 1) return hh_mc_accumulate(ctx, models, c, accum_dev, terminals ? terminals[0] : nullptr);
   HH_HIP(ctx, hipSetDevice(ctx->device));
   if (c->strategy == HH_BROADIE_KAYA) {
+    ctx->mirror_armed = 0;
     const uint32_t count = hh::bk_record_count(c->n_paths);
     if ((rc = ensure(ctx, ctx->records, ctx->records_cap, 2 * (size_t)count * hh::kRecStride))) return rc;
     std::vector<int> leader(n_models, -1);
@@ -574,6 +715,7 @@
   for (uint32_t k = 0; k < n_models; ++k) {
     p[k].records = (fuse ? ctx->frecords : ctx->records) + (size_t)k * rec_elems;
     p[k].accum = fuse ? accum_dev + (size_t)k * HH_ACC_LEN : nullptr;
+    p[k].accum_mirror = ctx->mirror_armed ? ctx->mirror_dev + (size_t)k * HH_ACC_LEN : nullptr;
     double* t = terminals ? terminals[k] : nullptr;
     p[k].terminal = !t ? nullptr : c->terminal_on_device ? t : ctx->terminal + (size_t)k * n_term;
   }
@@ -584,7 +726,8 @@
     if (!fuse)
       for (int k = 0; k < take; ++k)
         HH_HIP(ctx, hh::launch_reduce_records(p[k0 + k].records, hh::sim_records(*c), (double)c->n_paths,
-                                              accum_dev + (size_t)(k0 + k) * HH_ACC_LEN, ctx->stream, 1, &models[k0 + k], c));
+                                              accum_dev + (size_t)(k0 + k) * HH_ACC_LEN, ctx->stream, 1, &models[k0 + k], c,
+                                              false, nullptr, p[k0 + k].accum_mirror));
     k0 += (uint32_t)take;
   }
   if ((rc = end_timing(ctx))) return rc;
@@ -609,15 +752,15 @@
   const size_t n_acc = (size_t)n_models * HH_ACC_LEN;
   int rc = ensure(ctx, ctx->basket_accum, ctx->basket_accum_cap, n_acc);
   if (rc) return rc;
+  const Disarm disarm{ctx};
+  if ((rc = hh::arm_delivery(ctx, n_acc, terminals != nullptr))) return rc;
   HH_HIP(ctx, hipEventRecord(ctx->ev0, ctx->stream));
   if ((rc = hh_mc_accumulate_multi(ctx, models, n_models, c, ctx->basket_accum, terminals))) return rc;
   HH_HIP(ctx, hipEventRecord(ctx->ev1, ctx->stream));
-  double host[HH_MAX_MODELS * HH_ACC_LEN];
-  HH_HIP(ctx, hipMemcpyAsync(host, ctx->basket_accum, n_acc * sizeof(double), hipMemcpyDeviceToHost, ctx->stream));
-  HH_HIP(ctx, hipStreamSynchronize(ctx->stream));
+  if ((rc = hh::await_delivery(&ctx, 1, &ctx->basket_accum, n_acc, nullptr))) return rc;
   double kernel_ms, total_ms;
   if ((rc = solve_times(ctx, clock, &kernel_ms, &total_ms))) return rc;
-  rc = finalize_results(models, 1, c, host, n_models, kernel_ms, total_ms, out);
+  rc = finalize_results(models, 1, c, ctx->mirror, n_models, kernel_ms, total_ms, out);
   return rc ? finalize_failed(ctx, rc) : HH_OK;
 }
 
@@ -677,17 +820,16 @@
   const size_t n_acc = (size_t)n_payoffs * HH_ACC_LEN;
   int rc = ensure(ctx, ctx->basket_accum, ctx->basket_accum_cap, n_acc);
   if (rc) return rc;
+  const Disarm disarm{ctx};
+  if ((rc = hh::arm_delivery(ctx, n_acc, true))) return rc;
   HH_HIP(ctx, hipEventRecord(ctx->ev0, ctx->stream));
   rc = hh_mc_accumulate_basket(ctx, m, c, strikes, cps, n_payoffs, ctx->basket_accum, terminal);
   if (rc) return rc;
   HH_HIP(ctx, hipEventRecord(ctx->ev1, ctx->stream));
-  std::vector<double> host(n_acc);
-  HH_HIP(ctx, hipMemcpyAsync(host.data(), ctx->basket_accum, n_acc * sizeof(double),
-                             hipMemcpyDeviceToHost, ctx->stream));
-  HH_HIP(ctx, hipStreamSynchronize(ctx->stream));
+  if ((rc = hh::await_delivery(&ctx, 1, &ctx->basket_accum, n_acc, nullptr))) return rc;
   double kernel_ms, total_ms;
   if ((rc = solve_times(ctx, clock, &kernel_ms, &total_ms))) return rc;
-  rc = finalize_results(m, 0, c, host.data(), n_payoffs, kernel_ms, total_ms, out);
+  rc = finalize_results(m, 0, c, ctx->mirror, n_payoffs, kernel_ms, total_ms, out);
   return rc ? finalize_failed(ctx, rc) : HH_OK;
 }
 
@@ -725,14 +867,15 @@
   const WallClock clock;
   std::memset(out, 0, sizeof(*out));
   HH_HIP(ctx, hipSetDevice(ctx->device));
+  const Disarm disarm{ctx};
+  int rc = hh::arm_delivery(ctx, HH_ACC_LEN, terminal != nullptr);
+  if (rc) return rc;
   HH_HIP(ctx, hipEventRecord(ctx->ev0, ctx->stream));
-  int rc = hh_mc_accumulate(ctx, m, c, ctx->accum, terminal);
+  rc = hh_mc_accumulate(ctx, m, c, ctx->accum, terminal);
   if (rc) return rc;
   HH_HIP(ctx, hipEventRecord(ctx->ev1, ctx->stream));
-  HH_HIP(ctx, hipMemcpyAsync(ctx->accum_host, ctx->accum, HH_ACC_LEN * sizeof(double),
-                             hipMemcpyDeviceToHost, ctx->stream));
-  HH_HIP(ctx, hipStreamSynchronize(ctx->stream));
-  rc = hh_mc_finalize(m, c, ctx->accum_host, out);
+  if ((rc = hh::await_delivery(&ctx, 1, &ctx->accum, HH_ACC_LEN, nullptr))) return rc;
+  rc = hh_mc_finalize(m, c, ctx->mirror, out);
   if (rc) return finalize_failed(ctx, rc);
   return solve_times(ctx, clock, &out->kernel_ms, &out->total_ms);
 }
diff --git a/hedgehog.jl_amd/csrc/hh_bk.hip b/hedgehog.jl_amd/csrc/hh_bk.hip
--- a/hedgehog.jl_amd/csrc/hh_bk.hip
+++ b/hedgehog.jl_amd/csrc/hh_bk.hip
@@ -1080,7 +1080,8 @@
 
 __global__ __launch_bounds__(kTile) void bk_tail_kernel(const BkArgs* __restrict__ args, const BkTables* __restrict__ tabs,
                                                         uint32_t n_tiles, double n_paths, double* __restrict__ accum,
-                                                        uint32_t* __restrict__ cnt, const double* __restrict__ records) {
+                                                        uint32_t* __restrict__ cnt, const double* __restrict__ records,
+                                                        double* __restrict__ accum_mirror) {
   const uint32_t b = blockIdx.x, tid = threadIdx.x;
   __shared__ double sm[257];
   const uint32_t n_long_v = __hip_atomic_load(cnt, __ATOMIC_RELAXED, __HIP_MEMORY_SCOPE_AGENT);
@@ -1122,7 +1123,9 @@
     return;
   }
   if (tid == 0) {
-    accum[b] = b == (uint32_t)HH_ACC_NPATHS ? n_paths : out;
+    out = b == (uint32_t)HH_ACC_NPATHS ? n_paths : out;
+    accum[b] = out;
+    if (accum_mirror) __hip_atomic_store(accum_mirror + b, out, __ATOMIC_RELAXED, __HIP_MEMORY_SCOPE_SYSTEM);
     if (b == 0u) cnt[1] = n_rec;
   }
 }
@@ -1431,7 +1434,8 @@
   return v;
 }
 
-void bk_chain(const BkArgs& a0, const BkLayout& L, hipStream_t s, double* accum, double n_acc, int draw = 0) {
+void bk_chain(const BkArgs& a0, const BkLayout& L, hipStream_t s, double* accum, double n_acc, int draw = 0,
+              double* accum_mirror = nullptr) {
   BkArgs a = a0;
   const uint32_t resident = cf_resident_workgroups();
   a.drain_tile = resident != 0u && L.n_tiles > resident ? L.n_tiles - resident : 0xffffffffu;
@@ -1446,7 +1450,7 @@
   else
     hipLaunchKernelGGL(bk_cf_kernel<0>, g, b, 0, s, a, tabs);
   hipLaunchKernelGGL(bk_tail_kernel, dim3(kHeavyGrid), b, 0, s, static_cast<const BkArgs*>(a.args_dev), tabs, L.n_tiles,
-                     n_acc, accum, a.counters, static_cast<const double*>(a.records));
+                     n_acc, accum, a.counters, static_cast<const double*>(a.records), accum_mirror);
 }
 
 }
@@ -1472,7 +1476,7 @@
     hipLaunchKernelGGL(bk_draw_kernel, dim3(L.n_tiles), dim3(kTile), 0, s, a);
     draw = 0;
   }
-  bk_chain(a, L, s, ptr.accum, (double)c.n_paths, draw);
+  bk_chain(a, L, s, ptr.accum, (double)c.n_paths, draw, tr ? nullptr : ptr.accum_mirror);
   return (int)hipGetLastError();
 }
 
diff --git a/hedgehog.jl_amd/csrc/hh_ctx.h b/hedgehog.jl_amd/csrc/hh_ctx.h
--- a/hedgehog.jl_amd/csrc/hh_ctx.h
+++ b/hedgehog.jl_amd/csrc/hh_ctx.h
@@ -78,6 +78,11 @@
   uint64_t seed_clock = 0, seed_hits = 0, seed_uploads = 0, seed_evictions = 0;
   double* accum = nullptr;
   double* accum_host = nullptr;
+  double* mirror = nullptr;
+  double* mirror_dev = nullptr;
+  size_t mirror_cap = 0;
+  size_t mirror_armed = 0;
+  int result_delivery = HH_RESULT_DELIVERY_MIRROR;
   static constexpr int kTimingSlots = 256;
   bool timing = false;
   hipEvent_t tev[kTimingSlots][2] = {};
@@ -85,6 +90,11 @@
   char err[512] = {0};
   std::recursive_mutex mu;
 };
+
+namespace hh {
+int arm_delivery(hh_ctx* ctx, size_t n_words, bool by_copy);
+int await_delivery(hh_ctx* const* ctx, int n, double* const* dev, size_t n_words, int* bad);
+}
 
 namespace {
 
diff --git a/hedgehog.jl_amd/csrc/hh_kernels.h b/hedgehog.jl_amd/csrc/hh_kernels.h
--- a/hedgehog.jl_amd/csrc/hh_kernels.h
+++ b/hedgehog.jl_amd/csrc/hh_kernels.h
@@ -55,6 +55,7 @@
   unsigned long long finish_spin_ticks;
   uint32_t reducer_tile;
   PartialMap map;
+  double* accum_mirror;
 };
 
 struct DevicePtrs {
@@ -64,6 +65,7 @@
   double* terminal_d;
   double* records;
   double* accum;
+  double* accum_mirror;
   unsigned int* finish_state;
   long long finish_spin_ticks = -1;
   int finish_tile_first = 0;
@@ -139,7 +141,7 @@
 int launch_reduce_records(const double* records, uint32_t n_records, double n_paths, double* accum,
                           hipStream_t s, uint32_t n_groups = 1, const hh_model* m = nullptr,
                           const hh_config* c = nullptr, bool basket = false,
-                          const uint32_t* n_records_dev = nullptr);
+                          const uint32_t* n_records_dev = nullptr, double* accum_mirror = nullptr);
 int count_active_partials(const hh_model& m, const hh_config& c);
 int launch_basket_payoffs(const BasketArgs& b, uint32_t n_payoffs, uint32_t n_active_partials,
                           hipStream_t s);
diff --git a/hedgehog.jl_amd/csrc/hh_kernels.hip b/hedgehog.jl_amd/csrc/hh_kernels.hip
--- a/hedgehog.jl_amd/csrc/hh_kernels.hip
+++ b/hedgehog.jl_amd/csrc/hh_kernels.hip
@@ -294,7 +294,8 @@
                                                               uint32_t n, double n_paths,
                                                               double* __restrict__ accum,
                                                               const PartialMap map,
-                                                              const uint32_t* __restrict__ n_dev) {
+                                                              const uint32_t* __restrict__ n_dev,
+                                                              double* __restrict__ accum_mirror) {
   __shared__ double sm[257];
   const int slot = blockIdx.x;
   rec += (size_t)blockIdx.y * n * kRecStride;
@@ -315,7 +316,11 @@
   } else {
     out = sum_slot(rec, n, slot, sm);
   }
-  if (threadIdx.x == 0) accum[slot] = (slot == HH_ACC_NPATHS) ? n_paths : out;
+  if (threadIdx.x == 0) {
+    out = (slot == HH_ACC_NPATHS) ? n_paths : out;
+    accum[slot] = out;
+    if (accum_mirror) store_system(accum_mirror + (size_t)blockIdx.y * kRecStride + slot, out);
+  }
 }
 
 
@@ -469,6 +474,7 @@
   a.terminal_d = p.terminal_d;
   a.records = p.records;
   a.accum = p.accum;
+  a.accum_mirror = p.accum ? p.accum_mirror : nullptr;
   a.acc_n_paths = (double)c.n_paths;
   a.finish_state = p.finish_state;
   a.finish_spin_ticks = p.finish_spin_ticks < 0 ? kFinishSpinTicksDefault : (unsigned long long)p.finish_spin_ticks;
@@ -544,7 +550,7 @@
 
 int launch_reduce_records(const double* records, uint32_t n_records, double n_paths, double* accum,
                           hipStream_t s, uint32_t n_groups, const hh_model* m, const hh_config* c,
-                          bool basket, const uint32_t* n_records_dev) {
+                          bool basket, const uint32_t* n_records_dev, double* accum_mirror) {
   PartialMap pm{};
   if (m && c && (basket || c->strategy != HH_BROADIE_KAYA)) {
     if (c->n_partials) pm = classify_partials(*m, *c);
@@ -553,7 +559,7 @@
       for (double& d : pm.dK) d = 0.0;
   }
   hipLaunchKernelGGL(reduce_records_kernel, dim3(kRecStride, n_groups), dim3(256), 0, s, records,
-                     n_records, n_paths, accum, pm, n_records_dev);
+                     n_records, n_paths, accum, pm, n_records_dev, accum_mirror);
   return (int)hipGetLastError();
 }
 
diff --git a/hedgehog.jl_amd/csrc/hh_mgpu.hip b/hedgehog.jl_amd/csrc/hh_mgpu.hip
--- a/hedgehog.jl_amd/csrc/hh_mgpu.hip
+++ b/hedgehog.jl_amd/csrc/hh_mgpu.hip
@@ -289,6 +289,7 @@
     (void)hipSetDevice(mg->devices[g]);
     (void)hipStreamSynchronize(mg->ctx[g]->stream);
     mg->ctx[g]->shard.active = false;
+    mg->ctx[g]->mirror_armed = 0;
   }
   return rc;
 }
@@ -367,6 +368,11 @@
     const auto t0 = clk::now();
     hh_ctx* c = mg->ctx[g];
     HH_DHIP(mg, g, hipSetDevice(mg->devices[g]));
+    const bool by_copy = mg->mode == HH_MGPU_REDUCE_RCCL || (basket && !multi) || cfgs[g].n_paths == 0 || (terminals && terminals[g]);
+    if (const int r = hh::arm_delivery(c, n_acc, by_copy)) {
+      snprintf(mg->derr[g].data(), mg->derr[g].size(), "%s", hh_last_error(c));
+      return r;
+    }
     HH_DHIP(mg, g, hipEventRecord(c->ev0, c->stream));
     if (cfgs[g].n_paths == 0) {
       HH_DHIP(mg, g, hipMemsetAsync(mg->acc[g], 0, n_acc * sizeof(double), c->stream));
@@ -406,18 +412,16 @@
       }
     }
   }
-  if (!reduced) {
+  if (reduced) {
     for (int g = 0; g < mg->n; ++g) {
       HH_MHIP_DRAIN(mg, hipSetDevice(mg->devices[g]));
-      HH_MHIP_DRAIN(mg, hipMemcpyAsync(mg->host + (size_t)g * n_acc, mg->acc[g], n_acc * sizeof(double),
-                                       hipMemcpyDeviceToHost, mg->ctx[g]->stream));
-    }
-  }
-  for (int g = 0; g < mg->n; ++g) {
-    HH_MHIP_DRAIN(mg, hipSetDevice(mg->devices[g]));
-    HH_MHIP_DRAIN(mg, hipStreamSynchronize(mg->ctx[g]->stream));
-  }
-  if (!reduced) {
+      HH_MHIP_DRAIN(mg, hipStreamSynchronize(mg->ctx[g]->stream));
+    }
+  } else {
+    int bad = 0;
+    if ((rc = hh::await_delivery(mg->ctx.data(), mg->n, mg->acc.data(), n_acc, &bad)))
+      return drain(mg, mfail(mg, rc, "shard %d (device %d): %s", bad, mg->devices[bad], hh_last_error(mg->ctx[bad])));
+    for (int g = 0; g < mg->n; ++g) std::memcpy(mg->host + (size_t)g * n_acc, mg->ctx[g]->mirror, n_acc * sizeof(double));
     for (int g = 1; g < mg->n; ++g)
       for (size_t i = 0; i < n_acc; ++i) mg->host[i] += mg->host[(size_t)g * n_acc + i];
   }
diff --git a/hedgehog.jl_amd/csrc/hh_sim.h b/hedgehog.jl_amd/csrc/hh_sim.h
--- a/hedgehog.jl_amd/csrc/hh_sim.h
+++ b/hedgehog.jl_amd/csrc/hh_sim.h
@@ -229,6 +229,9 @@
 }
 __device__ __forceinline__ double load_through(const double* p) {
   return __hip_atomic_load(p, __ATOMIC_RELAXED, __HIP_MEMORY_SCOPE_AGENT);
+}
+__device__ __forceinline__ void store_system(double* p, double v) {
+  __hip_atomic_store(p, v, __ATOMIC_RELAXED, __HIP_MEMORY_SCOPE_SYSTEM);
 }
 __device__ __forceinline__ bool is_poison(double v) {
   return (unsigned long long)__double_as_longlong(v) == kPoison;
@@ -424,7 +427,9 @@
     }
     if (slot == HH_ACC_NPATHS) out = n_paths;
     const bool dirty = scalar_load_end(state_in_flight) != 0u;
-    accum[slot] = (gave_up || dirty) ? __longlong_as_double(0x7FF8000000000000ll) : out;
+    out = (gave_up || dirty) ? __longlong_as_double(0x7FF8000000000000ll) : out;
+    accum[slot] = out;
+    if (a.accum_mirror) store_system(a.accum_mirror + slot, out);
     if (slot == 0 && gave_up) __hip_atomic_store(a.finish_state, 1u, __ATOMIC_RELAXED, __HIP_MEMORY_SCOPE_AGENT);
   }
 }
diff --git a/include/hedgehog_mc.h b/include/hedgehog_mc.h
--- a/include/hedgehog_mc.h
+++ b/include/hedgehog_mc.h
@@ -104,7 +104,8 @@
 const char* hh_last_error(const hh_ctx* ctx);
 enum hh_option { HH_OPT_LSM_FORM = 1, HH_OPT_BK_TERM_CACHE = 2, HH_OPT_GRID_FORM = 3, HH_OPT_LSM_SPIN_TICKS = 4,
                  HH_OPT_FUSE_REDUCE = 5, HH_OPT_GRID_ORDER = 6, HH_OPT_FINISH_SPIN_TICKS = 7,
-                 HH_OPT_FINISH_TILE_FIRST = 8 };
+                 HH_OPT_FINISH_TILE_FIRST = 8, HH_OPT_RESULT_DELIVERY = 9 };
+enum hh_result_delivery { HH_RESULT_DELIVERY_COPY = 0, HH_RESULT_DELIVERY_MIRROR = 1 };
 enum hh_grid_form { HH_GRID_FORM_PER_DATE = 0, HH_GRID_FORM_BATCHED = 1 };
 enum hh_lsm_form { HH_LSM_FORM_PER_DATE = 0, HH_LSM_FORM_PERSISTENT = 1, HH_LSM_FORM_AUTO = 2 };
 int hh_ctx_set_option(hh_ctx* ctx, int32_t option, int64_t value);
```

After: 431.0 billion. 0.983x the previous value.
